# Chrissie-Law/Causal-Domain-Clustering-for-Multi-Domain-Recommendation

Hardware: AMD Instinct MI355X
Metric: train samples/sec + AUC parity, PLE 3-domain batch 4096 at 1/2/4/8 MI355X (higher is better)
Workload: dtype bf16; 1 GPU; PLE 3-domain full training step (fwd + BCE + whole-table L2 + bwd + Adam), 26 fields x vocab 1000000, emb_dim=16, batch 4096/GPU; global_batch=4096, table_mode=lazy, hip_graph=True, row_sort_one_batch_ahead=True, id_dist=uniform, parallelism=dp1, attention_branch=False, full=False, steady_state=True, preroll_steps=1785, flush_every=64

## Files before the change

causal-domain-clustering-for-multi-domain-recommendation_amd/_lib.py:

```python
import ctypes as C
import os

from . import build as _build

MAX_GROUPS = 32
MAX_TENSORS = 48
MAX_GATES = 16
MAX_SEL = 16
MAX_BN_SEGS = 24
SORT_MAX_B = 16384
SORT_MAX_ROWS = 32768
BN_ROWS_PER_BLOCK = 64
ROWDOT_PARTS = 256
PREC_BF16 = 0
PREC_F32 = 1

c_f = C.c_float
c_d = C.c_double
c_i32 = C.c_int32
c_i64 = C.c_int64
c_p = C.c_void_p


class AdamHP(C.Structure):
# ... 176 lines not shown

class MidBExpert2(C.Structure):
    _fields_ = [("wt", c_p), ("ldwt", c_i64), ("src", c_i32), ("pad_", c_i32)]


class MidBGate2(C.Structure):
    _fields_ = [("d_out", c_p), ("ld_dout", c_i64), ("probs", c_p), ("d_logits", c_p), ("ld_dlogits", c_i64),
                ("d_logits_h", c_p), ("ld_dlogits_h", c_i64), ("wt", c_p), ("ldwt", c_i64), ("src", c_i32), ("n_sel", c_i32),
                ("sel", c_i32 * MAX_SEL)]


class CgcMidBwdArgs(C.Structure):
    _fields_ = [("B", c_i64), ("H1", c_i32), ("H2", c_i32), ("n_exp1", c_i32), ("n_gate1", c_i32), ("n_exp2", c_i32), ("n_gate2", c_i32),
                ("ex1", c_p), ("ld_ex1", c_i64), ("ex2", c_p), ("ld_ex2", c_i64), ("dz1_h", c_p), ("ld_dz1_h", c_i64),
                ("dz2_h", c_p), ("ld_dz2_h", c_i64), ("mask1", c_i32), ("mask2", c_i32), ("scale1", c_f), ("scale2", c_f),
                ("g1", MidBGate1 * MID_MAX_GATE), ("e2", MidBExpert2 * MID_MAX_EXPERT), ("g2", MidBGate2 * MID_MAX_GATE)]


BN_X_BF16, BN_Y_BF16, BN_DY_BF16 = 1, 2, 4


class BnSeg(C.Structure):
    _fields_ = [("x", c_p), ("ldx", c_i64), ("y", c_p), ("ldy", c_i64), ("gamma", c_p), ("beta", c_p),
                ("running_mean", c_p), ("running_var", c_p), ("save_mean", c_p), ("save_invstd", c_p),
                ("num_batches_tracked", c_p), ("yh", c_p), ("ldyh", c_i64), ("C", c_i32), ("row_group", c_i32),
                ("half", c_i32), ("pad_", c_i32)]


class BnFwdArgs(C.Structure):
    _fields_ = [("n_seg", c_i32), ("training", c_i32), ("relu", c_i32), ("skip_le1", c_i32), ("eps", c_f), ("momentum", c_f),
                ("drop_p", c_f), ("seed", C.c_uint64), ("seed_offset_dev", c_p), ("M", c_i64),
                ("row_offsets", c_p), ("workspace", c_p), ("phase", c_i32), ("stats_ready", c_i32), ("exchange", c_p),
                ("s", BnSeg * MAX_BN_SEGS)]


class BnBSeg(C.Structure):
    _fields_ = [("dy", c_p), ("lddy", c_i64), ("y", c_p), ("ldy", c_i64), ("x", c_p), ("ldx", c_i64),
                ("dx", c_p), ("lddx", c_i64), ("gamma", c_p), ("save_mean", c_p), ("save_invstd", c_p),
                ("dgamma", c_p), ("dbeta", c_p), ("dxh", c_p), ("lddxh", c_i64), ("C", c_i32), ("row_group", c_i32), ("accumulate_dx", c_i32),
                ("half", c_i32)]


class BnBwdArgs(C.Structure):
    _fields_ = [("n_seg", c_i32), ("training", c_i32), ("relu", c_i32), ("eps", c_f), ("mask_scale", c_f),
                ("M", c_i64), ("row_offsets", c_p), ("workspace", c_p), ("phase", c_i32), ("pad_", c_i32), ("exchange", c_p),
                ("s", BnBSeg * MAX_BN_SEGS)]


class RowdotGroup(C.Structure):
    _fields_ = [("x", c_p), ("ldx", c_i64), ("w", c_p), ("bias", c_p), ("out", c_p), ("ld_out", c_i64),
                ("logit", c_p), ("ld_logit", c_i64), ("K", c_i32)]


class RowdotFwdArgs(C.Structure):
    _fields_ = [("n_groups", c_i32), ("sigmoid", c_i32), ("n_addend", c_i32), ("addend", c_p * 4),
                ("ld_addend", c_i64 * 4), ("M", c_i64), ("row_offsets", c_p), ("g", RowdotGroup * MAX_GROUPS)]


class RowdotBGroup(C.Structure):
    _fields_ = [("dout", c_p), ("ld_dout", c_i64), ("out", c_p), ("ld_out", c_i64), ("x", c_p), ("ldx", c_i64),
                ("w", c_p), ("dx", c_p), ("lddx", c_i64), ("dw", c_p), ("dbias", c_p), ("dlogit", c_p),
                ("ld_dlogit", c_i64), ("K", c_i32), ("accumulate_dx", c_i32)]


class RowdotBwdArgs(C.Structure):
    _fields_ = [("n_groups", c_i32), ("sigmoid", c_i32), ("M", c_i64), ("row_offsets", c_p), ("workspace", c_p),
                ("bce_group", c_p), ("bce_y_i16", c_p), ("bce_y_f32", c_p), ("bce_loss", c_p), ("bce_partial", c_p),
                ("bce_inv_count", c_f), ("pad_", c_i32), ("g", RowdotBGroup * MAX_GROUPS)]


HEAD_MAX_TOWERS = 8


class HeadTower(C.Structure):
    _fields_ = [("x", c_p), ("ldx", c_i64), ("w", c_p), ("bias", c_p), ("dx", c_p), ("lddx", c_i64), ("dw", c_p), ("dbias", c_p),
                ("K", c_i32), ("accumulate_dx", c_i32)]


class HeadArgs(C.Structure):
    _fields_ = [("n_tower", c_i32), ("sigmoid", c_i32), ("n_addend", c_i32), ("pad_", c_i32), ("M", c_i64),
                ("out", c_p), ("ld_out", c_i64), ("d_out", c_p), ("ld_dout", c_i64),
                ("wide_x", c_p), ("ld_wide", c_i64), ("wide_w", c_p), ("wide_bias", c_p), ("wide_out", c_p), ("ld_wide_out", c_i64),
                ("wide_dx", c_p), ("ld_wide_dx", c_i64), ("wide_dw", c_p), ("wide_dbias", c_p), ("wide_K", c_i32), ("accumulate_wide_dx", c_i32),
                ("addend", c_p * 2), ("ld_addend", c_i64 * 2), ("d_addend", c_p * 2), ("ld_d_addend", c_i64 * 2),
                ("accumulate_d_addend", c_i32 * 2), ("workspace", c_p),
                ("bce_group", c_p), ("bce_y_i16", c_p), ("bce_y_f32", c_p), ("bce_loss", c_p), ("bce_partial", c_p),
                ("bce_inv_count", c_f), ("pad2_", c_i32), ("t", HeadTower * HEAD_MAX_TOWERS)]


TOWER_MAX = 4
TOWER_ROWS = 128
TOWER_ERR_TIMEOUT = 0x40000000


class TowerLayer(C.Structure):
    _fields_ = [("wh", c_p), ("ldwh", c_i64), ("wt", c_p), ("ldwt", c_i64), ("bias", c_p), ("z", c_p), ("ldz", c_i64),
                ("dzh", c_p), ("lddzh", c_i64), ("gamma", c_p), ("beta", c_p), ("running_mean", c_p), ("running_var", c_p),
                ("num_batches_tracked", c_p), ("save_mean", c_p), ("save_invstd", c_p), ("dgamma", c_p), ("dbeta", c_p)]


class TowerDesc(C.Structure):
    _fields_ = [("xh", c_p), ("ldxh", c_i64), ("dx", c_p), ("lddx", c_i64), ("accumulate_dx", c_i32), ("pad_", c_i32),
                ("l1", TowerLayer), ("l2", TowerLayer), ("a1h", c_p), ("lda1h", c_i64), ("a2", c_p), ("lda2", c_i64),
                ("wo", c_p), ("bo", c_p), ("dwo", c_p), ("dbo", c_p), ("dy2", c_p), ("lddy2", c_i64), ("dy1", c_p), ("lddy1", c_i64)]


class TowerArgs(C.Structure):
    _fields_ = [("n_tower", c_i32), ("H0", c_i32), ("H1", c_i32), ("H2", c_i32), ("M", c_i64), ("relu", c_i32), ("sigmoid", c_i32),
                ("drop_p", c_f), ("eps", c_f), ("momentum", c_f), ("pad_", c_i32), ("seed1", C.c_uint64), ("seed2", C.c_uint64),
                ("seed_offset_dev", c_p), ("out", c_p), ("ld_out", c_i64), ("d_out", c_p), ("ld_dout", c_i64),
                ("wide_x", c_p), ("ld_wide", c_i64), ("wide_w", c_p), ("wide_bias", c_p), ("wide_dx", c_p), ("ld_wide_dx", c_i64),
                ("wide_dw", c_p), ("wide_dbias", c_p), ("wide_K", c_i32), ("accumulate_wide_dx", c_i32),
                ("bce_group", c_p), ("bce_y_i16", c_p), ("bce_y_f32", c_p), ("bce_loss", c_p), ("bce_inv_count", c_f), ("pad2_", c_i32),
                ("workspace", c_p), ("err", c_p), ("exchange", c_p * 4), ("t", TowerDesc * TOWER_MAX)]


class StarFuseArgs(C.Structure):
    _fields_ = [("n", c_i32), ("op", c_i32), ("size", c_i64), ("s", c_p), ("ds", c_p), ("accumulate_ds", c_i32), ("pad_", c_i32),
                ("a", c_p * MAX_GROUPS), ("out", c_p * MAX_GROUPS), ("da", c_p * MAX_GROUPS)]


class AdamTensor(C.Structure):
    _fields_ = [("w", c_p), ("g", c_p), ("m", c_p), ("v", c_p), ("n", c_i64), ("l2", c_f), ("n_slabs", c_i32), ("slabs", c_p),
                ("slab_stride", c_i64)]


class AddNArgs(C.Structure):
    _fields_ = [("dst", c_p), ("ld_dst", c_i64), ("rows", c_i64), ("cols", c_i32), ("n", c_i32), ("accumulate", c_i32),
                ("src", c_p * MAX_GROUPS), ("ld_src", c_i64 * MAX_GROUPS)]


class AdamArgs(C.Structure):
    _fields_ = [("n_tensors", c_i32), ("lerp_w", c_f), ("beta2", c_f), ("one_minus_beta2", c_f), ("eps", c_f),
                ("weight_decay", c_f), ("step_scalars", c_p), ("n_scalars", c_i32), ("grad_scale", c_f),
                ("step_dev", c_p), ("reg_sum", c_p), ("reg_seed", c_p), ("t", AdamTensor * MAX_TENSORS)]


_SIGNATURES = {
    "cdc_abi_version": (c_i32, []),
    "cdc_last_error": (C.c_char_p, []),
    "cdc_embed_gather_fwd": (c_i32, [c_p, c_p, c_p, c_p, c_p, c_p, c_i64, c_i32, c_i32, c_i64, c_p]),
    "cdc_embed_gather_fwd_h": (c_i32, [c_p, c_p, c_p, c_p, c_p, c_i64, c_p, c_p, c_i64, c_i32, c_i32, c_i64, c_p]),
    "cdc_embed_index": (c_i32, [c_p, c_p, c_p, c_p, c_i64, c_i32, c_i64, c_p]),
    "cdc_embed_sort_dedupe": (c_i32, [c_p, c_p, c_p, c_p, c_p, c_p, c_i64, c_i32, c_p]),
    "cdc_embed_sort_dedupe_ids": (c_i32, [c_p, c_p, c_i64, c_p, c_p, c_i32, c_p, c_p, c_p, c_p, c_p, c_p, c_i64, c_i32, c_p]),
    "cdc_embed_segment_sum": (c_i32, [c_p, c_p, c_p, c_p, c_p, c_p, c_i64, c_i32, c_i32, c_p]),
    "cdc_embed_segment_sum_direct": (c_i32, [c_p, c_p, c_p, c_p, c_p, c_p, c_i64, c_i32, c_i32, c_p]),
    "cdc_embed_segsum_lazy_update": (c_i32, [c_p, c_p, c_p, c_p, c_p, c_p, c_p, c_p, c_p, AdamHP, c_p, c_i64, c_i32, c_i32, c_i32, c_p]),
    "cdc_embed_grad_dense": (c_i32, [c_p, c_p, c_p, c_p, c_i64, c_i32, c_i32, c_i64, c_p]),
    "cdc_embed_adam_touched": (c_i32, [c_p, c_p, c_p, c_p, c_p, c_p, c_p, AdamHP, c_p, c_i64, c_i32, c_i32, c_p]),
    "cdc_embed_adam_dense_pass": (c_i32, [c_p, c_p, c_p, c_i64, AdamHP, c_p, c_p, c_p]),
    "cdc_embed_adam_patch": (c_i32, [c_p, c_p, c_p, c_p, c_p, c_p, c_i64, c_i32, c_i32, c_p]),
    "cdc_embed_lazy_catchup": (c_i32, [c_p, c_p, c_p, c_p, c_p, c_p, AdamHP, c_p, c_p, c_i32, c_i64, c_i32, c_i32, c_p]),
    "cdc_embed_lazy_catchup_gather": (c_i32, [c_p, c_p, c_p, c_p, c_p, c_p, c_p, c_p, AdamHP, c_p, c_p, c_p, c_i64, c_i64, c_i32, c_i32, c_p]),
    "cdc_embed_lazy_update": (c_i32, [c_p, c_p, c_p, c_p, c_p, c_p, c_p, AdamHP, c_p, c_p, c_i32, c_i64, c_i32, c_i32, c_p]),
    "cdc_embed_lazy_flush": (c_i32, [c_p, c_p, c_p, c_p, c_i64, c_i32, AdamHP, c_p, c_i32, c_i32, c_i32, c_i32, c_p]),
    "cdc_embed_lazy_flush_bg": (c_i32, [c_p, c_p, c_p, c_p, c_i64, c_i32, AdamHP, c_p, c_i32, c_i32, c_i32, c_i32, c_i32, c_p]),
    "cdc_embed_merge_dedupe": (c_i32, [c_p, c_p, c_p, c_p, c_p, c_p, c_i64, c_i32, c_i32, c_p]),
    "cdc_eval_workspace_bytes": (c_i64, [c_i64, c_i32]),
    "cdc_eval_metrics": (c_i32, [c_p, c_p, c_p, c_i64, c_i64, c_i32, c_p, c_p, c_p, c_p, c_i64, c_p]),
    "cdc_eval_gauc_workspace_bytes": (c_i64, [c_i64, c_i32, c_i64]),
    "cdc_eval_gauc": (c_i32, [c_p, c_p, c_p, c_i64, c_i64, c_p, c_i64, c_i32, c_p, c_i64, c_p, c_p, c_p, c_p, c_i64, c_p]),
    "cdc_eval_auc_delong_workspace_bytes": (c_i64, [c_i64, c_i32, c_i32]),
    "cdc_eval_auc_delong": (c_i32, [c_p, c_p, c_p, c_p, c_i64, c_i64, c_i32, c_p, c_p, c_p, c_p, c_i64, c_p]),
    "cdc_eval_loss_ci_workspace_bytes": (c_i64, [c_i64, c_i32, c_i32]),
    "cdc_eval_loss_ci": (c_i32, [c_p, c_p, c_p, c_p, c_i64, c_i64, c_i32, c_p, c_p, c_p, c_p, c_i64, c_p]),
    "cdc_eval_gauc_ci_workspace_bytes": (c_i64, [c_i64, c_i32, c_i64, c_i32]),
    "cdc_eval_gauc_ci": (c_i32, [c_p, c_p, c_p, c_p, c_i64, c_i64, c_p, c_i64, c_i32, c_p, c_i64, c_p, c_p, c_p, c_p, c_i64, c_p]),
    "cdc_eval_bootstrap_workspace_bytes": (c_i64, [c_i64, c_i32, c_i64, c_i32, c_i32]),
    "cdc_eval_bootstrap": (c_i32, [c_p, c_p, c_p, c_p, c_i64, c_i64, c_p, c_i64, c_i32, c_p, c_i64, c_i32, C.c_uint64, c_i32, c_p, c_p, c_p,
                                   c_p, c_i64, c_p]),
    "cdc_eval_calibration_bootstrap_workspace_bytes": (c_i64, [c_i64, c_i32, c_i32, c_i32, c_i32]),
    "cdc_eval_calibration_bootstrap": (c_i32, [c_p, c_p, c_p, c_p, c_i64, c_i64, c_p, c_i64, c_i32, c_i32, c_i64, c_i32, C.c_uint64, c_p,
                                               c_p, c_p, c_p, c_i64, c_p]),
    "cdc_eval_calibration_workspace_bytes": (c_i64, [c_i64, c_i32, c_i32]),
    "cdc_eval_calibration": (c_i32, [c_p, c_p, c_p, c_i64, c_i64, c_i32, c_i32, c_p, c_p, c_p, c_p, c_p, c_p, c_p, c_i64, c_p]),
    "cdc_eval_isotonic_max_blocks": (c_i64, [c_i64, c_i32]),
    "cdc_eval_isotonic_fit_workspace_bytes": (c_i64, [c_i64, c_i32]),
    "cdc_eval_isotonic_fit": (c_i32, [c_p, c_p, c_p, c_i64, c_i64, c_i32, c_p, c_p, c_p, c_p, c_p, c_p, c_i64, c_p, c_p, c_p, c_p, c_i64, c_p]),
    "cdc_eval_isotonic_apply": (c_i32, [c_p, c_p, c_i64, c_i64, c_i32, c_p, c_p, c_p, c_p, c_p, c_f, c_p, c_p, c_p]),
    "cdc_eval_platt_fit_workspace_bytes": (c_i64, [c_i64, c_i32]),
    "cdc_eval_platt_fit": (c_i32, [c_p, c_p, c_p, c_i64, c_i64, c_i32, c_i32, c_i32, c_d, c_d, c_i32, c_p, c_p, c_p, c_p, c_p, c_p, c_p, c_p, c_p, c_p,
                                   c_p, c_i64, c_p]),
    "cdc_eval_platt_apply": (c_i32, [c_p, c_p, c_i64, c_i64, c_i32, c_p, c_p, c_p, c_i32, c_d, c_f, c_p, c_p, c_p]),
    "cdc_eval_segments": (c_i32, [c_p, c_i64, c_p, c_p, c_i32, c_p, c_p, c_p, c_p, c_p, c_i64, c_i32, c_p]),
    "cdc_shard_bucket": (c_i32, [c_p, c_p, c_p, c_p, c_p, c_i64, c_i32, c_i32, c_i32, c_p]),
    "cdc_shard_expand": (c_i32, [c_p, c_p, c_p, c_p, c_p, c_p, c_p, c_i64, c_i32, c_i32, c_i32, c_i32, c_p]),
    "cdc_shard_pack": (c_i32, [c_p, c_p, c_p, c_p, c_p, c_i64, c_i32, c_i32, c_i32, c_i32, c_p]),
    "cdc_glinear_fwd": (c_i32, [C.POINTER(LinFwdArgs), c_i32, c_p]),
    "cdc_glinear_bwd_x": (c_i32, [C.POINTER(LinBwdxArgs), c_i32, c_p]),
    "cdc_transpose_multi": (c_i32, [C.POINTER(TransposeArgs), c_p]),
    "cdc_gemm_bf16_nt": (c_i32, [C.POINTER(G2Args), c_p]),
    "cdc_weight_shadows": (c_i32, [C.POINTER(WShadowArgs), c_p]),
    "cdc_shadow_bf16": (c_i32, [C.POINTER(ShadowArgs), c_p]),
    "cdc_glinear_bwd_w": (c_i32, [C.POINTER(LinBwdwArgs), c_i32, c_p]),
    "cdc_glinear_bwd_w_pair": (c_i32, [C.POINTER(LinBwdwArgs), C.POINTER(LinBwdwArgs), c_p, c_p]),
    "cdc_glinear_bwd_w_pair_reduce": (c_i32, [C.POINTER(LinBwdwArgs), C.POINTER(LinBwdwArgs), c_p, c_p]),
    "cdc_gate_pool_fwd": (c_i32, [C.POINTER(PoolFwdArgs), c_p]),
    "cdc_cgc_mid_fwd": (c_i32, [C.POINTER(CgcMidFwdArgs), c_p]),
    "cdc_cgc_mid_bwd": (c_i32, [C.POINTER(CgcMidBwdArgs), c_p]),
    "cdc_cgc_mid_fits": (c_i32, [c_i32, c_i32, c_i32, c_i32]),
    "cdc_expert_pair_fwd": (c_i32, [C.POINTER(ExpertPairArgs), c_p]),
    "cdc_gate_pool_bwd": (c_i32, [C.POINTER(PoolBwdArgs), c_p]),
    "cdc_gate_pool_wide_table": (c_i32, [c_i32, c_i32, c_p, c_p, c_p, c_i64]),
    "cdc_gate_pool_wide_fwd": (c_i32, [C.POINTER(PoolWideFwdArgs), c_p]),
    "cdc_gate_pool_wide_bwd": (c_i32, [C.POINTER(PoolWideBwdArgs), c_p]),
    "cdc_bn_fwd": (c_i32, [C.POINTER(BnFwdArgs), c_p]),
    "cdc_bn_bwd": (c_i32, [C.POINTER(BnBwdArgs), c_p]),
    "cdc_rowdot_fwd": (c_i32, [C.POINTER(RowdotFwdArgs), c_p]),
    "cdc_rowdot_bwd": (c_i32, [C.POINTER(RowdotBwdArgs), c_p]),
    "cdc_head_fwd": (c_i32, [C.POINTER(HeadArgs), c_p]),
    "cdc_head_bwd": (c_i32, [C.POINTER(HeadArgs), c_p]),
    "cdc_head_workspace_floats": (c_i64, [C.POINTER(HeadArgs)]),
    "cdc_tower_fwd": (c_i32, [C.POINTER(TowerArgs), c_p]),
    "cdc_tower_bwd": (c_i32, [C.POINTER(TowerArgs), c_p]),
    "cdc_tower_step": (c_i32, [C.POINTER(TowerArgs), c_p]),
    "cdc_tower_workspace_bytes": (c_i64, [C.POINTER(TowerArgs)]),
    "cdc_tower_dp": (c_i32, [C.POINTER(TowerArgs), c_i32, c_p]),
    "cdc_bce_fwd_bwd": (c_i32, [c_p, c_i64, c_p, c_p, c_p, c_p, c_p, c_i64, c_i64, c_i32, c_f, c_p]),
    "cdc_attn_fwd": (c_i32, [c_p, c_i64, c_p, c_i64, c_p, c_i64, c_i32, c_i32, c_i32, c_f, C.c_uint64, c_p, c_p]),
    "cdc_attn_bwd": (c_i32, [c_p, c_i64, c_p, c_p, c_i64, c_p, c_i64, c_i64, c_i32, c_i32, c_i32, c_f, C.c_uint64, c_p, c_p]),
    "cdc_add_relu_fwd": (c_i32, [c_p, c_i64, c_p, c_i64, c_p, c_i64, c_i64, c_i32, c_p]),
    "cdc_add_relu_bwd": (c_i32, [c_p, c_i64, c_p, c_i64, c_p, c_i64, c_i32, c_p, c_i64, c_i32, c_i64, c_i32, c_p]),
    "cdc_sigmoid_gate_fwd": (c_i32, [c_p, c_i64, c_p, c_i64, c_p, c_i64, c_i64, c_i32, c_f, c_f, c_f, c_p]),
    "cdc_sigmoid_gate_bwd": (c_i32, [c_p, c_i64, c_p, c_i64, c_p, c_i64, c_p, c_i64, c_i32, c_p, c_i64, c_i32, c_i64, c_i32, c_f, c_f, c_f, c_p]),
    "cdc_group_select_fwd": (c_i32, [c_p, c_i64, c_p, c_p, c_i64, c_i64, c_i32, c_i32, c_p]),
    "cdc_group_select_bwd": (c_i32, [c_p, c_i64, c_p, c_p, c_i64, c_i64, c_i32, c_i32, c_i32, c_p]),
    "cdc_stage_batch": (c_i32, [c_p, c_p, c_p, c_p, c_p, c_p, c_i64, c_i32, c_p, c_p, c_p]),
    "cdc_stage_batch_next": (c_i32, [c_p, c_p, c_p, c_p, c_p, c_p, c_i64, c_i32, c_p, c_p, c_p, c_p, c_i32, c_p, c_p, c_p]),
    "cdc_fm_fwd": (c_i32, [c_p, c_i64, c_p, c_i64, c_i64, c_i32, c_i32, c_p]),
    "cdc_fm_bwd": (c_i32, [c_p, c_i64, c_p, c_i64, c_p, c_i64, c_i64, c_i32, c_i32, c_i32, c_p]),
    "cdc_bce_mean_fwd_bwd": (c_i32, [c_p, c_i64, c_p, c_p, c_p, c_p, c_i64, c_i64, c_i32, c_f, c_p]),
    "cdc_cross_fwd": (c_i32, [c_p, c_i64, c_p, c_i64, c_p, c_p, c_p, c_i64, c_p, c_i64, c_i32, c_p]),
    "cdc_cross_bwd": (c_i32, [c_p, c_i64, c_p, c_i64, c_p, c_i64, c_p, c_p, c_p, c_i64, c_p, c_i64, c_p, c_p, c_p, c_i64, c_i32, c_p]),
    "cdc_tanh_fwd": (c_i32, [c_p, c_i64, c_p, c_i64, c_i64, c_i32, c_p]),
    "cdc_tanh_bwd": (c_i32, [c_p, c_i64, c_p, c_i64, c_p, c_i64, c_i64, c_i32, c_i32, c_p]),
    "cdc_cross_combine_fwd": (c_i32, [c_p, c_i64, c_p, c_i64, c_p, c_p, c_p, c_i64, c_p, c_i64, c_i64, c_i32, c_i32, c_p]),
    "cdc_cross_combine_bwd": (c_i32, [c_p, c_i64, c_p, c_i64, c_p, c_i64, c_p, c_p, c_i64, c_p, c_i64, c_p, c_i64, c_i32,
                                      c_p, c_i32, c_p, c_i32, c_p, c_i64, c_i32, c_i32, c_p]),
    "cdc_add_out": (c_i32, [c_p, c_i64, c_p, c_i64, c_p, c_i64, c_i64, c_i32, c_p]),
    "cdc_copy_or_add": (c_i32, [c_p, c_i64, c_p, c_i64, c_i64, c_i32, c_i32, c_p]),
    "cdc_star_fuse_fwd": (c_i32, [C.POINTER(StarFuseArgs), c_p]),
    "cdc_star_fuse_bwd": (c_i32, [C.POINTER(StarFuseArgs), c_p]),
    "cdc_sum_slices": (c_i32, [c_p, c_i64, c_p, c_i64, c_i64, c_i32, c_i32, c_i32, c_p]),
    "cdc_adam_multi": (c_i32, [C.POINTER(AdamArgs), c_p]),
    "cdc_adam_multi_table": (c_i32, [C.POINTER(AdamArgs), c_p, c_p, c_p, c_i32, c_p]),
    "cdc_embed_segsum_lazy_update_dense": (c_i32, [c_p, c_p, c_p, c_p, c_p, c_p, c_p, c_p, c_p, AdamHP, c_p, c_i64, c_i32, c_i32, c_i32,
                                                   C.POINTER(AdamArgs), c_p, c_p, c_p, c_i32, c_p]),
    "cdc_step_increment": (c_i32, [c_p, c_p]),
    "cdc_begin_step": (c_i32, [c_p, c_p, c_i32, c_p]),
    "cdc_fill_f32": (c_i32, [c_p, c_f, c_i64, c_p]),
    "cdc_fill_f64": (c_i32, [c_p, C.c_double, c_i64, c_p]),
    "cdc_add_inplace": (c_i32, [c_p, c_i64, c_p, c_i64, c_i64, c_i32, c_p]),
    "cdc_add_n": (c_i32, [c_p, c_p]),
    "cdc_mul_bcast": (c_i32, [c_p, c_p, c_p, c_i64, c_i64, c_p]),
    "cdc_mul_bcast_bwd": (c_i32, [c_p, c_p, c_p, c_p, c_p, c_i64, c_i64, c_p]),
    "cdc_group_partition": (c_i32, [c_p, c_p, c_p, c_i64, c_i32, c_p]),
    "cdc_rows_permute": (c_i32, [c_p, c_i64, c_p, c_p, c_i64, c_i64, c_i32, c_i32, c_p]),
}

_lib = None


class HipExtensionError(RuntimeError):
    pass


def lib_path():
    return _build.LIB_PATH


def load():
    global _lib
    if _lib is not None:
        return _lib
    path = _build.LIB_PATH
    if not _build.is_fresh():
        try:
            _build.build(verbose=False)
        except Exception as e:
            if not os.path.exists(path):
                raise HipExtensionError(
                    f"libcdcmdr.so is missing at {path} and could not be built ({e}); "
                    "run `python __graft_entry__.py build` — there is no CPU fallback") from e
            import warnings
            warnings.warn(f"libcdcmdr.so is older than its sources and the rebuild failed: {str(e)[:400]}")
    try:
        lib = C.CDLL(path)
    except OSError as e:
        raise HipExtensionError(f"cannot load {path}: {e}; there is no CPU fallback") from e
    for name, (res, args) in _SIGNATURES.items():
        try:
            fn = getattr(lib, name)
        except AttributeError as e:
            raise HipExtensionError(f"{path} does not export {name}") from e
        fn.restype = res
        fn.argtypes = args
    if lib.cdc_abi_version() != 1:
        raise HipExtensionError(f"ABI version mismatch: library {lib.cdc_abi_version()} != binding 1")
    _lib = lib
    return lib


def exported_symbols():
    return sorted(_SIGNATURES)


def check(rc, what):
    if rc != 0:
        msg = load().cdc_last_error()
        raise RuntimeError(f"{what} failed (rc={rc}): {msg.decode() if msg else ''}")


PROFILE = None
TRACE = os.environ.get("CDC_TRACE_LAUNCH") == "1"


def launch(name, fn, args, stream, flops=0.0, nbytes=0.0):
    if TRACE:
        import sys
        sys.stderr.write(f"[cdc launch] {name}\n")
        sys.stderr.flush()
    if PROFILE is None:
        rc = fn(*args, stream)
    else:
        import torch
        e0, e1 = torch.cuda.Event(enable_timing=True), torch.cuda.Event(enable_timing=True)
        e0.record()
        rc = fn(*args, stream)
        e1.record()
        PROFILE.append((name, e0, e1, flops, nbytes))
    if rc != 0:
        check(rc, name)
```

causal-domain-clustering-for-multi-domain-recommendation_amd/csrc/embedding.hip:

```cpp
#include "common.h"
#include "adam_dense.h"

template <int VEC>
__global__ void __launch_bounds__(256) k_gather_fwd(const int32_t* __restrict__ ids, const int32_t* __restrict__ offsets,
                                                    const float* __restrict__ table, float* __restrict__ out,
                                                    __bf16* __restrict__ out_h, int64_t ld_out_h,
                                                    int32_t* __restrict__ idx_out, int32_t* __restrict__ err_flag,
                                                    int64_t n_pos, int32_t F, int32_t D, int64_t R) {
    CDC_PRIO_MAIN();
    const int chunks = D / VEC;
    const int64_t total = n_pos * chunks;
    for (int64_t i = (int64_t)blockIdx.x * blockDim.x + threadIdx.x; i < total; i += (int64_t)gridDim.x * blockDim.x) {
        const int64_t pos = i / chunks;
        const int c = (int)(i - pos * chunks);
        const int f = (int)(pos % F);
        const int32_t row = (int32_t)((uint32_t)ids[pos] + (uint32_t)offsets[f]);
        const bool ok = row >= 0 && (int64_t)row < R;
        if (c == 0 && idx_out) idx_out[pos] = ok ? row : -1;
        if (!ok && c == 0 && err_flag) atomicMax(err_flag, (int32_t)(pos < 0x7ffffffe ? pos + 1 : 0x7fffffff));
        if (VEC == 4) {
            float4 val = make_float4(0.f, 0.f, 0.f, 0.f);
            if (ok) val = *reinterpret_cast<const float4*>(table + (int64_t)row * D + c * 4);
            *reinterpret_cast<float4*>(out + pos * D + c * 4) = val;
            if (out_h) {
// ... 406 lines not shown
static int sort_raise_lds_limit(const char* who) {
    static bool attr_set = false;
    if (attr_set) return 0;
    const void* const kernels[] = {(const void*)k_sort_dedupe, (const void*)k_sort_chunk, (const void*)k_merge_lds<uint64_t, false>,
                                   (const void*)k_merge_lds<uint32_t, true>};
    for (const void* k : kernels) {
        const hipError_t e = hipFuncSetAttribute(k, hipFuncAttributeMaxDynamicSharedMemorySize, 160 * 1024);
        if (e != hipSuccess) { cdc_set_error("%s: cannot raise LDS limit: %s", who, hipGetErrorString(e)); return (int)e; }
    }
    attr_set = true;
    return 0;
}
static int merge_lanes(const char* who, int n_runs, int& P) {
    P = 1;
    while (P < n_runs) P <<= 1;
    CDC_CHECK_ARG(P <= 64, CDC_E_TOOBIG, "%s: %d runs", who, n_runs);
    return 0;
}
static int dedupe_merged_launch(const uint64_t* merged, int32_t* uniq_row, int32_t* seg_start, int32_t* perm, int32_t* uniq_cnt, int64_t B,
                                int32_t F, hipStream_t st) {
    hipLaunchKernelGGL(k_dedupe_merged, dim3(F), dim3(SORT_THREADS), 0, st, merged, uniq_row, seg_start, perm, uniq_cnt, (int32_t)B, F);
    CDC_LAUNCH_CHECK("embed_dedupe_merged");
    return 0;
}

static int sort_dedupe_launch(const SortSrc& src, int32_t* uniq_row, int32_t* seg_start, int32_t* perm, int32_t* uniq_cnt,
                              uint64_t* scratch, int64_t B, int32_t F, void* stream) {
    const int32_t* idx = src.idx;
    CDC_CHECK_ARG(idx && uniq_row && seg_start && perm && uniq_cnt, CDC_E_BADARG, "embed_sort_dedupe: null pointer");
    CDC_CHECK_ARG(B > 0 && F > 0, CDC_E_BADARG, "embed_sort_dedupe: bad sizes");
    CDC_CHECK_ARG(B <= CDC_SORT_MAX_ROWS, CDC_E_TOOBIG, "embed_sort_dedupe: B=%ld exceeds %d", (long)B, CDC_SORT_MAX_ROWS);
    CDC_CHECK_ARG(scratch || B <= SORT_CHUNK, CDC_E_BADARG, "embed_sort_dedupe: B > %d needs a scratch buffer of 2*F*B uint64", SORT_CHUNK);
    if (const int rc = sort_raise_lds_limit("embed_sort_dedupe")) return rc;
    hipStream_t st = (hipStream_t)stream;
    if (B > 1024 && B <= SORT_RADIX_MAX) {
        hipLaunchKernelGGL(k_sort_dedupe_radix, dim3(F), dim3(SORT_THREADS), 0, st, src, uniq_row, seg_start, perm, uniq_cnt, (int32_t)B, F);
        CDC_LAUNCH_CHECK("embed_sort_dedupe_radix");
        return 0;
    }
    if (B <= 1024 || (!scratch && B <= SORT_CHUNK)) {
        int n_pad = SORT_THREADS;
        while (n_pad < B) n_pad <<= 1;
        const size_t lds = (size_t)n_pad * 8 + SORT_THREADS * 4;
        hipLaunchKernelGGL(k_sort_dedupe, dim3(F), dim3(SORT_THREADS), lds, st, src, uniq_row, seg_start, perm, uniq_cnt, (int32_t)B, F, n_pad);
        CDC_LAUNCH_CHECK("embed_sort_dedupe");
        return 0;
    }
    int chunk = 512;
    while (chunk < SORT_CHUNK && (int64_t)chunk * 8 < B) chunk <<= 1;
    const int n_runs = (int)cdc_ceil_div(B, chunk);
    uint64_t* runs = scratch;
    uint64_t* merged = scratch + (int64_t)F * B;
    hipLaunchKernelGGL(k_sort_chunk, dim3(F, n_runs), dim3(SORT_THREADS), (size_t)chunk * 8, st, src, runs, (int32_t)B, F, chunk);
    CDC_LAUNCH_CHECK("embed_sort_chunk");
    int P;
    if (const int rc = merge_lanes("embed_sort_dedupe", n_runs, P)) return rc;
    if ((size_t)B * 8 <= MERGE_LDS_MAX) {
        hipLaunchKernelGGL((k_merge_lds<uint64_t, false>), dim3(F, n_runs), dim3(SORT_THREADS), (size_t)B * 8, st, runs, merged, (int32_t)B, F,
                           n_runs, chunk, P);
    } else {
        const int64_t blocks = cdc_ceil_div((int64_t)F * B * P, 256);
        hipLaunchKernelGGL(k_merge_runs, dim3((unsigned)blocks), dim3(256), 0, st, runs, merged, (int32_t)B, F, chunk, n_runs, P);
    }
    CDC_LAUNCH_CHECK("embed_merge_runs");
    return dedupe_merged_launch(merged, uniq_row, seg_start, perm, uniq_cnt, B, F, st);
}

extern "C" int cdc_embed_sort_dedupe(const int32_t* idx, int32_t* uniq_row, int32_t* seg_start, int32_t* perm,
                                     int32_t* uniq_cnt, uint64_t* scratch, int64_t B, int32_t F, void* stream) {
    const SortSrc src = {idx, nullptr, 0, nullptr, nullptr, 0, nullptr};
    return sort_dedupe_launch(src, uniq_row, seg_start, perm, uniq_cnt, scratch, B, F, stream);
}
extern "C" int cdc_embed_sort_dedupe_ids(const int32_t* ids, const int32_t* offsets, int64_t R, int32_t* step_dev, double* accumulators,
                                         int32_t n_acc, int32_t* err_flag, int32_t* uniq_row, int32_t* seg_start, int32_t* perm,
                                         int32_t* uniq_cnt, uint64_t* scratch, int64_t B, int32_t F, void* stream) {
    CDC_CHECK_ARG(offsets && R > 0 && n_acc >= 0 && n_acc <= 64 && (n_acc == 0 || accumulators) && (step_dev || n_acc == 0), CDC_E_BADARG,
                  "embed_sort_dedupe_ids: bad argument");
    const SortSrc src = {ids, offsets, R, step_dev, accumulators, n_acc, err_flag};
    return sort_dedupe_launch(src, uniq_row, seg_start, perm, uniq_cnt, scratch, B, F, stream);
}

extern "C" int cdc_embed_merge_dedupe(const int32_t* idx, int32_t* uniq_row, int32_t* seg_start, int32_t* perm, int32_t* uniq_cnt,
                                      uint64_t* scratch, int64_t B, int32_t F, int32_t n_runs, void* stream) {
    CDC_CHECK_ARG(idx && uniq_row && seg_start && perm && uniq_cnt && scratch, CDC_E_BADARG, "embed_merge_dedupe: null pointer");
    CDC_CHECK_ARG(B > 0 && F > 0 && n_runs > 0 && B % n_runs == 0, CDC_E_BADARG, "embed_merge_dedupe: bad sizes");
    CDC_CHECK_ARG(B <= CDC_SORT_MAX_ROWS, CDC_E_TOOBIG, "embed_merge_dedupe: B=%ld exceeds %d", (long)B, CDC_SORT_MAX_ROWS);
    hipStream_t st = (hipStream_t)stream;
    int P;
    if (const int rc = merge_lanes("embed_merge_dedupe", n_runs, P)) return rc;
    if (const int rc = sort_raise_lds_limit("embed_merge_dedupe")) return rc;
    static_assert((size_t)CDC_SORT_MAX_ROWS * 4 <= MERGE_LDS_MAX, "cdc_embed_merge_dedupe stages a whole field in LDS");
    hipLaunchKernelGGL((k_merge_lds<uint32_t, true>), dim3(F, n_runs), dim3(SORT_THREADS), (size_t)B * 4, st, idx, scratch, (int32_t)B, F,
                       n_runs, (int32_t)(B / n_runs), P);
    CDC_LAUNCH_CHECK("embed_merge_n");
    return dedupe_merged_launch(scratch, uniq_row, seg_start, perm, uniq_cnt, B, F, st);
}

struct RowItem {
    int64_t slot, row;
    int f, j, d;
    bool live;
};
template <int VEC, bool ROW = true>
__device__ __forceinline__ RowItem row_item(int64_t i, int chunks, int B, const int32_t* __restrict__ uniq_cnt,
                                            const int32_t* __restrict__ uniq_row) {
    RowItem it;
    it.d = (int)(i % chunks) * VEC;
    it.slot = i / chunks;
    it.f = (int)(it.slot / B);
    it.j = (int)(it.slot - (int64_t)it.f * B);
    it.row = -1;
    it.live = it.j < uniq_cnt[it.f];
    if (ROW && it.live) {
        it.row = uniq_row[it.slot];
        it.live = it.row >= 0;
    }
    return it;
}
template <int VEC>
__device__ __forceinline__ void load_wmv(const float* w, const float* m, const float* v, int64_t e0, float (&wv)[VEC], float (&mv)[VEC],
                                         float (&vv)[VEC]) {
    if (VEC == 4) {
        const float4 a4 = *reinterpret_cast<const float4*>(w + e0), b4 = *reinterpret_cast<const float4*>(m + e0),
                     c4 = *reinterpret_cast<const float4*>(v + e0);
        wv[0] = a4.x; wv[1 % VEC] = a4.y; wv[2 % VEC] = a4.z; wv[3 % VEC] = a4.w;
        mv[0] = b4.x; mv[1 % VEC] = b4.y; mv[2 % VEC] = b4.z; mv[3 % VEC] = b4.w;
        vv[0] = c4.x; vv[1 % VEC] = c4.y; vv[2 % VEC] = c4.z; vv[3 % VEC] = c4.w;
    } else {
        wv[0] = w[e0]; mv[0] = m[e0]; vv[0] = v[e0];
    }
}
template <int VEC>
__device__ __forceinline__ void store_wmv(float* w, float* m, float* v, int64_t e0, const float (&wv)[VEC], const float (&mv)[VEC],
                                          const float (&vv)[VEC]) {
    if (VEC == 4) {
        *reinterpret_cast<float4*>(w + e0) = make_float4(wv[0], wv[1 % VEC], wv[2 % VEC], wv[3 % VEC]);
        *reinterpret_cast<float4*>(m + e0) = make_float4(mv[0], mv[1 % VEC], mv[2 % VEC], mv[3 % VEC]);
        *reinterpret_cast<float4*>(v + e0) = make_float4(vv[0], vv[1 % VEC], vv[2 % VEC], vv[3 % VEC]);
    } else {
        w[e0] = wv[0]; m[e0] = mv[0]; v[e0] = vv[0];
    }
}
template <int VEC>
__device__ __forceinline__ void row_adam_step(float* w, float* m, float* v, int32_t* last, int64_t row, int D, int d0, const float (&g)[VEC],
                                              const AdamConsts& c, float step_size, float bc2s, int32_t t) {
    const int64_t e0 = row * D + d0;
    float wv[VEC], mv[VEC], vv[VEC];
    load_wmv<VEC>(w, m, v, e0, wv, mv, vv);
#pragma unroll
    for (int q = 0; q < VEC; ++q) adam_elem(wv[q], mv[q], vv[q], g[q], c, step_size, bc2s);
    store_wmv<VEC>(w, m, v, e0, wv, mv, vv);
    if (d0 == 0) last[row] = t;
}

#define SEG_SPLIT 64
#define SEG_DIRECT 8
#define SEG_BLOCK 512
#define SEG_LONG_BLOCKS 64
#define SEG_LIST_CAP (CDC_SORT_MAX_ROWS / SEG_LONG_BLOCKS)

struct SegSink {
    float* rowgrad;
    float* w; float* m; float* v;
    int32_t* last;
    const int32_t* uniq_row;
    AdamConsts c;
    float step_size, bc2s;
    int32_t t;
};
template <int VEC>
__device__ __forceinline__ void seg_finish(const SegSink& k, int64_t slot, int D, int d0, const float (&acc)[VEC]) {
    if (!k.w) {
        float* dst = k.rowgrad + slot * D + d0;
        if (VEC == 4) *reinterpret_cast<float4*>(dst) = make_float4(acc[0], acc[1 % VEC], acc[2 % VEC], acc[3 % VEC]);
        else dst[0] = acc[0];
        return;
    }
    const int64_t row = k.uniq_row[slot];
    if (row < 0) return;
    row_adam_step<VEC>(k.w, k.m, k.v, k.last, row, D, d0, acc, k.c, k.step_size, k.bc2s, k.t);
}
__device__ __forceinline__ SegSink seg_sink_store(float* rowgrad) {
    SegSink k = {};
    k.rowgrad = rowgrad;
    return k;
}

template <int VEC>
__device__ __forceinline__ void seg_direct_body(int bid, int nblocks, const float* __restrict__ d_out, const int32_t* __restrict__ seg_start,
                                                const int32_t* __restrict__ perm, const int32_t* __restrict__ uniq_cnt,
                                                const int32_t* __restrict__ uniq_row, const SegSink& sink,
                                                int32_t B, int32_t F, int32_t D, int32_t max_len) {
    const int chunks = D / VEC;
    const int64_t total = (int64_t)F * B * chunks;
    for (int64_t i = (int64_t)bid * blockDim.x + threadIdx.x; i < total; i += (int64_t)nblocks * blockDim.x) {
        const RowItem it = row_item<VEC, false>(i, chunks, B, uniq_cnt, nullptr);
        if (!it.live) continue;
        if (uniq_row && uniq_row[it.slot] < 0) continue;
        const int f = it.f, j = it.j;
        const int32_t* sst = seg_start + (int64_t)f * (B + 1);
        const int32_t* prm = perm + (int64_t)f * B;
        const int k0 = sst[j], k1 = sst[j + 1];
        if (max_len > 0 && k1 - k0 >= max_len) continue;
        float acc[VEC];
#pragma unroll
        for (int q = 0; q < VEC; ++q) acc[q] = 0.f;
        for (int k = k0; k < k1; k += 8) {
            int p[8];
            float v[8][VEC];
#pragma unroll
            for (int q = 0; q < 8; ++q) p[q] = (k + q < k1) ? prm[k + q] : -1;
#pragma unroll
            for (int q = 0; q < 8; ++q) {
                const float* src = d_out + ((int64_t)(p[q] >= 0 ? p[q] : 0) * F + f) * D + it.d;
                if (p[q] >= 0) {
                    if (VEC == 4) {
                        const float4 t = *reinterpret_cast<const float4*>(src);
                        v[q][0] = t.x; v[q][1] = t.y; v[q][2] = t.z; v[q][3] = t.w;
                    } else {
                        v[q][0] = src[0];
                    }
                }
            }
#pragma unroll
            for (int q = 0; q < 8; ++q)
                if (p[q] >= 0) {
#pragma unroll
                    for (int e = 0; e < VEC; ++e) acc[e] = __fadd_rn(acc[e], v[q][e]);
                }
        }
        seg_finish<VEC>(sink, it.slot, D, it.d, acc);
    }
}
template <int VEC>
__global__ void __launch_bounds__(256) k_segment_sum_direct(const float* __restrict__ d_out, const int32_t* __restrict__ seg_start,
                                                            const int32_t* __restrict__ perm, const int32_t* __restrict__ uniq_cnt,
                                                            const int32_t* __restrict__ uniq_row, float* __restrict__ rowgrad,
                                                            int32_t B, int32_t F, int32_t D, int32_t max_len) {
    seg_direct_body<VEC>(blockIdx.x, gridDim.x, d_out, seg_start, perm, uniq_cnt, uniq_row, seg_sink_store(rowgrad), B, F, D, max_len);
}
extern "C" int cdc_embed_segment_sum_direct(const float* d_out, const int32_t* seg_start, const int32_t* perm,
                                            const int32_t* uniq_cnt, const int32_t* uniq_row, float* rowgrad, int64_t B, int32_t F,
                                            int32_t D, void* stream) {
    CDC_CHECK_ARG(d_out && seg_start && perm && uniq_cnt && rowgrad, CDC_E_BADARG, "embed_segment_sum_direct: null pointer");
    CDC_CHECK_ARG(B > 0 && F > 0 && D > 0 && B <= CDC_SORT_MAX_ROWS, CDC_E_BADARG, "embed_segment_sum_direct: bad sizes");
    const bool vec = (D % 4 == 0) && (((uintptr_t)d_out | (uintptr_t)rowgrad) % 16 == 0);
    int blocks = (int)std::min<int64_t>(cdc_ceil_div((int64_t)F * B * (vec ? D / 4 : D), 256), 8192);
    if (vec)
        hipLaunchKernelGGL(k_segment_sum_direct<4>, dim3(blocks), dim3(256), 0, (hipStream_t)stream, d_out, seg_start, perm, uniq_cnt, uniq_row,
                           rowgrad, (int32_t)B, F, D, 0);
    else
        hipLaunchKernelGGL(k_segment_sum_direct<1>, dim3(blocks), dim3(256), 0, (hipStream_t)stream, d_out, seg_start, perm, uniq_cnt, uniq_row,
                           rowgrad, (int32_t)B, F, D, 0);
    CDC_LAUNCH_CHECK("embed_segment_sum_direct");
    return 0;
}

template <int BATCH = 16>
__device__ __forceinline__ float seg_serial_sum(const float* __restrict__ d_out, const int32_t* __restrict__ prm, int begin, int end,
                                                int F, int D, int f, int d) {
    float acc = 0.f;
    for (int k = begin; k < end; k += BATCH) {
        int p[BATCH];
        float x[BATCH];
#pragma unroll
        for (int q = 0; q < BATCH; ++q) p[q] = (k + q < end) ? prm[k + q] : -1;
#pragma unroll
        for (int q = 0; q < BATCH; ++q) x[q] = p[q] >= 0 ? d_out[((int64_t)p[q] * F + f) * D + d] : 0.f;
#pragma unroll
        for (int q = 0; q < BATCH; ++q)
            if (p[q] >= 0) acc = __fadd_rn(acc, x[q]);
    }
    return acc;
}
template <int VEC>
__device__ __forceinline__ void seg_long_body(int f, int by, const float* __restrict__ d_out, const int32_t* __restrict__ seg_start,
                                              const int32_t* __restrict__ perm, const int32_t* __restrict__ uniq_cnt,
                                              const SegSink& sink, int32_t B, int32_t F, int32_t D, int32_t subs,
                                              int32_t min_len) {
    __shared__ int32_t list[SEG_LIST_CAP];
    __shared__ int32_t n_list;
    __shared__ __attribute__((aligned(16))) float parts[256 * VEC];
    const int tid = threadIdx.x, lane = tid & 63, wave = tid >> 6;
    const int n = uniq_cnt[f];
    const int32_t* sst = seg_start + (int64_t)f * (B + 1);
    const int32_t* prm = perm + (int64_t)f * B;
    if (tid == 0) n_list = 0;
    __syncthreads();
    for (int j = by + SEG_LONG_BLOCKS * tid; j < n; j += SEG_LONG_BLOCKS * 256)
        if (sst[j + 1] - sst[j] >= min_len) list[atomicAdd(&n_list, 1)] = j;
    __syncthreads();
    const int count = n_list;
    if (count == 0) return;
    const bool block_rows = subs > 1;
    for (int i = wave; i < count; i += 4) {
        const int j = list[i];
        const int k0 = sst[j], len = sst[j + 1] - k0;
        if (block_rows && len >= SEG_BLOCK) continue;
        const int64_t slot = (int64_t)f * B + j;
        if (subs <= 1) {
            for (int d = lane; d < D; d += 64) {
                const float one[1] = {seg_serial_sum(d_out, prm + k0, 0, len, F, D, f, d)};
                seg_finish<1>(sink, slot, D, d, one);
            }
            continue;
        }
        const int sub = lane / D, d = lane - sub * D;
        const bool split = len >= SEG_SPLIT;
        int begin = 0, end = (sub == 0) ? len : 0;
        if (split) {
            const int q = (len + subs - 1) / subs;
            begin = min(sub * q, len);
            end = min(begin + q, len);
        }
        float acc = seg_serial_sum(d_out, prm + k0, begin, end, F, D, f, d);
        if (split) {
            float total = __shfl(acc, d, 64);
            for (int s2 = 1; s2 < subs; ++s2) total = __fadd_rn(total, __shfl(acc, s2 * D + d, 64));
            acc = total;
        }
        if (sub == 0) {
            const float one[1] = {acc};
            seg_finish<1>(sink, slot, D, d, one);
        }
    }
    if (!block_rows) return;
    const int chunks = D / VEC;
    const int P = 256 / chunks;
    const int part = tid / chunks, d = (tid - part * chunks) * VEC;
    for (int i = 0; i < count; ++i) {
        const int j = list[i];
        const int k0 = sst[j], len = sst[j + 1] - k0;
        if (len < SEG_BLOCK) continue;
        const int q = (len + P - 1) / P;
        const int begin = min(part * q, len), end = min(begin + q, len);
        float acc[VEC];
#pragma unroll
        for (int e = 0; e < VEC; ++e) acc[e] = 0.f;
        if (part < P) {
            constexpr int NB = VEC == 4 ? 16 : 32;
            for (int k = begin; k < end; k += NB) {
                int pr[NB];
#pragma unroll
                for (int u = 0; u < NB; ++u) pr[u] = (k + u < end) ? prm[k0 + k + u] : -1;
                float x[NB][VEC];
#pragma unroll
                for (int u = 0; u < NB; ++u) {
                    if (pr[u] >= 0) {
                        const float* src = d_out + ((int64_t)pr[u] * F + f) * D + d;
                        if (VEC == 4) {
                            const float4 t4 = *reinterpret_cast<const float4*>(src);
                            x[u][0] = t4.x; x[u][1 % VEC] = t4.y; x[u][2 % VEC] = t4.z; x[u][3 % VEC] = t4.w;
                        } else {
                            x[u][0] = src[0];
                        }
                    }
                }
#pragma unroll
                for (int u = 0; u < NB; ++u)
                    if (pr[u] >= 0) {
#pragma unroll
                        for (int e = 0; e < VEC; ++e) acc[e] = __fadd_rn(acc[e], x[u][e]);
                    }
            }
        }
#pragma unroll
        for (int e = 0; e < VEC; ++e) parts[tid * VEC + e] = acc[e];
        __syncthreads();
        if (tid < chunks) {
            float total[VEC];
#pragma unroll
            for (int e = 0; e < VEC; ++e) total[e] = parts[tid * VEC + e];
            for (int p2 = 1; p2 < P; ++p2)
#pragma unroll
                for (int e = 0; e < VEC; ++e) total[e] = __fadd_rn(total[e], parts[(p2 * chunks + tid) * VEC + e]);
            seg_finish<VEC>(sink, (int64_t)f * B + j, D, tid * VEC, total);
        }
        __syncthreads();
    }
}

template <int VEC>
__global__ void __launch_bounds__(256) k_segment_sum(const float* __restrict__ d_out, const int32_t* __restrict__ seg_start,
                                                     const int32_t* __restrict__ perm, const int32_t* __restrict__ uniq_cnt,
                                                     SegSink sink, cdc_adam_hp hp, const int32_t* __restrict__ step_dev, int32_t B,
                                                     int32_t F, int32_t D, int32_t subs) {
    if (sink.w) {
        sink.c = make_consts(hp);
        sink.t = *step_dev;
        step_scalars_at(hp.step_scalars, hp.n_scalars, sink.t, sink.step_size, sink.bc2s);
    }
    const int n_long = F * SEG_LONG_BLOCKS;
    if ((int)blockIdx.x < n_long)
        seg_long_body<VEC>(blockIdx.x / SEG_LONG_BLOCKS, blockIdx.x % SEG_LONG_BLOCKS, d_out, seg_start, perm, uniq_cnt, sink, B, F, D,
                           subs, SEG_DIRECT);
    else
        seg_direct_body<VEC>(blockIdx.x - n_long, gridDim.x - n_long, d_out, seg_start, perm, uniq_cnt, nullptr, sink, B, F, D, SEG_DIRECT);
}
template <int VEC>
__global__ void __launch_bounds__(256, 4) k_segment_sum_dense(const float* __restrict__ d_out, const int32_t* __restrict__ seg_start,
                                                           const int32_t* __restrict__ perm, const int32_t* __restrict__ uniq_cnt,
                                                           SegSink sink, cdc_adam_hp hp, const int32_t* __restrict__ step_dev, int32_t B,
                                                           int32_t F, int32_t D, int32_t subs, const AdamHdr h,
                                                           const cdc_adam_tensor* __restrict__ tab, const int32_t* __restrict__ wg_tensor,
                                                           const int32_t* __restrict__ wg_chunk, int32_t n_dense, int32_t short_only) {
    const int n_long = short_only ? 0 : F * SEG_LONG_BLOCKS;
    const int b = (int)blockIdx.x;
    if (b >= n_long && b < n_long + n_dense) {
        const int ti = __builtin_amdgcn_readfirstlane(wg_tensor[b - n_long]);
        const int chunk = __builtin_amdgcn_readfirstlane(wg_chunk[b - n_long]);
        const cdc_adam_tensor T = tab[ti];
        adam_chunk<ADAM_CHUNK / 2>(h, T, chunk, b == n_long);
        return;
    }
    sink.c = make_consts(hp);
    sink.t = *step_dev;
    step_scalars_at(hp.step_scalars, hp.n_scalars, sink.t, sink.step_size, sink.bc2s);
    if (b < n_long)
        seg_long_body<VEC>(b / SEG_LONG_BLOCKS, b % SEG_LONG_BLOCKS, d_out, seg_start, perm, uniq_cnt, sink, B, F, D, subs, SEG_DIRECT);
    else
        seg_direct_body<VEC>(b - n_long - n_dense, (int)gridDim.x - n_long - n_dense, d_out, seg_start, perm, uniq_cnt,
                             short_only ? sink.uniq_row : nullptr, sink, B, F, D, short_only ? 0 : SEG_DIRECT);
}
template <int VEC>
__global__ void __launch_bounds__(256) k_segment_sum_short_sink(const float* __restrict__ d_out, const int32_t* __restrict__ seg_start,
                                                                const int32_t* __restrict__ perm, const int32_t* __restrict__ uniq_cnt,
                                                                SegSink sink, cdc_adam_hp hp, const int32_t* __restrict__ step_dev,
                                                                int32_t B, int32_t F, int32_t D) {
    sink.c = make_consts(hp);
    sink.t = *step_dev;
    step_scalars_at(hp.step_scalars, hp.n_scalars, sink.t, sink.step_size, sink.bc2s);
    seg_direct_body<VEC>(blockIdx.x, gridDim.x, d_out, seg_start, perm, uniq_cnt, sink.uniq_row, sink, B, F, D, 0);
}

struct SegGeom {
    bool vec;
    int direct_blocks, subs;
    SegSink sink;
};
static SegGeom seg_geometry(const float* d_out, float* rowgrad, float* w, float* m, float* v, int32_t* last, const int32_t* uniq_row,
                            int64_t B, int32_t F, int32_t D) {
    SegGeom g = {};
    g.vec = (D % 4 == 0) && (((uintptr_t)d_out | (uintptr_t)rowgrad | (uintptr_t)w | (uintptr_t)m | (uintptr_t)v) % 16 == 0);
    g.direct_blocks = (int)std::min<int64_t>(cdc_ceil_div((int64_t)F * B * (g.vec ? D / 4 : D), 256), 8192);
    g.subs = (D <= 64 && 64 % D == 0) ? 64 / D : 1;
    g.sink.rowgrad = rowgrad;
    g.sink.w = w; g.sink.m = m; g.sink.v = v; g.sink.last = last; g.sink.uniq_row = uniq_row;
    return g;
}

extern "C" int cdc_embed_segment_sum(const float* d_out, const int32_t* seg_start, const int32_t* perm,
                                     const int32_t* uniq_cnt, float* sorted_scratch, float* rowgrad, int64_t B, int32_t F,
                                     int32_t D, void* stream) {
    (void)sorted_scratch;
    CDC_CHECK_ARG(d_out && seg_start && perm && uniq_cnt && rowgrad, CDC_E_BADARG, "embed_segment_sum: null pointer");
    CDC_CHECK_ARG(B > 0 && F > 0 && D > 0 && B <= CDC_SORT_MAX_ROWS, CDC_E_BADARG, "embed_segment_sum: bad sizes");
    hipStream_t st = (hipStream_t)stream;
    const SegGeom g = seg_geometry(d_out, rowgrad, nullptr, nullptr, nullptr, nullptr, nullptr, B, F, D);
    const int blocks = g.direct_blocks + F * SEG_LONG_BLOCKS;
    const cdc_adam_hp no_hp = {};
    if (g.vec) hipLaunchKernelGGL(k_segment_sum<4>, dim3(blocks), dim3(256), 0, st, d_out, seg_start, perm, uniq_cnt, g.sink, no_hp, nullptr, (int32_t)B, F, D, g.subs);
    else       hipLaunchKernelGGL(k_segment_sum<1>, dim3(blocks), dim3(256), 0, st, d_out, seg_start, perm, uniq_cnt, g.sink, no_hp, nullptr, (int32_t)B, F, D, g.subs);
    CDC_LAUNCH_CHECK("embed_segment_sum");
    return 0;
}

extern "C" int cdc_embed_segsum_lazy_update(const float* d_out, const int32_t* seg_start, const int32_t* perm, const int32_t* uniq_cnt,
                                            const int32_t* uniq_row, float* w, float* m, float* v, int32_t* last, cdc_adam_hp hp,
                                            const int32_t* step_dev, int64_t B, int32_t F, int32_t D, int32_t short_only, void* stream) {
    CDC_CHECK_ARG(d_out && seg_start && perm && uniq_cnt && uniq_row && w && m && v && last && step_dev && hp.step_scalars &&
                      hp.n_scalars > 0, CDC_E_BADARG, "embed_segsum_lazy_update: null pointer");
    CDC_CHECK_ARG(B > 0 && F > 0 && D > 0 && B <= CDC_SORT_MAX_ROWS, CDC_E_BADARG, "embed_segsum_lazy_update: bad sizes");
    hipStream_t st = (hipStream_t)stream;
    const SegGeom g = seg_geometry(d_out, nullptr, w, m, v, last, uniq_row, B, F, D);
    if (short_only) {
        if (g.vec) hipLaunchKernelGGL(k_segment_sum_short_sink<4>, dim3(g.direct_blocks), dim3(256), 0, st, d_out, seg_start, perm, uniq_cnt, g.sink, hp, step_dev, (int32_t)B, F, D);
        else       hipLaunchKernelGGL(k_segment_sum_short_sink<1>, dim3(g.direct_blocks), dim3(256), 0, st, d_out, seg_start, perm, uniq_cnt, g.sink, hp, step_dev, (int32_t)B, F, D);
    } else {
        const int blocks = g.direct_blocks + F * SEG_LONG_BLOCKS;
        if (g.vec) hipLaunchKernelGGL(k_segment_sum<4>, dim3(blocks), dim3(256), 0, st, d_out, seg_start, perm, uniq_cnt, g.sink, hp, step_dev, (int32_t)B, F, D, g.subs);
        else       hipLaunchKernelGGL(k_segment_sum<1>, dim3(blocks), dim3(256), 0, st, d_out, seg_start, perm, uniq_cnt, g.sink, hp, step_dev, (int32_t)B, F, D, g.subs);
    }
    CDC_LAUNCH_CHECK("embed_segsum_lazy_update");
    return 0;
}

extern "C" int cdc_embed_segsum_lazy_update_dense(const float* d_out, const int32_t* seg_start, const int32_t* perm, const int32_t* uniq_cnt,
                                                  const int32_t* uniq_row, float* w, float* m, float* v, int32_t* last, cdc_adam_hp hp,
                                                  const int32_t* step_dev, int64_t B, int32_t F, int32_t D, int32_t short_only,
                                                  const cdc_adam_args* dense, const cdc_adam_tensor* tensors_dev, const int32_t* wg_tensor_dev,
                                                  const int32_t* wg_chunk_dev, int32_t n_dense_workgroups, void* stream) {
    CDC_CHECK_ARG(d_out && seg_start && perm && uniq_cnt && uniq_row && w && m && v && last && step_dev && hp.step_scalars &&
                      hp.n_scalars > 0, CDC_E_BADARG, "embed_segsum_lazy_update_dense: null pointer");
    CDC_CHECK_ARG(B > 0 && F > 0 && D > 0 && B <= CDC_SORT_MAX_ROWS, CDC_E_BADARG, "embed_segsum_lazy_update_dense: bad sizes");
    CDC_CHECK_ARG(dense && tensors_dev && wg_tensor_dev && wg_chunk_dev && n_dense_workgroups > 0 && n_dense_workgroups < (1 << 24) &&
                      dense->step_dev && dense->step_scalars && dense->n_scalars > 0, CDC_E_BADARG,
                  "embed_segsum_lazy_update_dense: the dense parameters' descriptor table (as for cdc_adam_multi_table) is missing");
    hipStream_t st = (hipStream_t)stream;
    const SegGeom g = seg_geometry(d_out, nullptr, w, m, v, last, uniq_row, B, F, D);
    const int blocks = g.direct_blocks + (short_only ? 0 : F * SEG_LONG_BLOCKS) + n_dense_workgroups;
    const AdamHdr h = {dense->lerp_w, dense->beta2, dense->one_minus_beta2, dense->eps, dense->weight_decay, dense->grad_scale,
                       dense->step_scalars, dense->n_scalars, dense->step_dev, dense->reg_sum, dense->reg_seed};
    if (g.vec) hipLaunchKernelGGL(k_segment_sum_dense<4>, dim3(blocks), dim3(256), 0, st, d_out, seg_start, perm, uniq_cnt, g.sink, hp, step_dev, (int32_t)B, F, D, g.subs,
                                  h, tensors_dev, wg_tensor_dev, wg_chunk_dev, n_dense_workgroups, short_only);
    else       hipLaunchKernelGGL(k_segment_sum_dense<1>, dim3(blocks), dim3(256), 0, st, d_out, seg_start, perm, uniq_cnt, g.sink, hp, step_dev, (int32_t)B, F, D, g.subs,
                                  h, tensors_dev, wg_tensor_dev, wg_chunk_dev, n_dense_workgroups, short_only);
    CDC_LAUNCH_CHECK("embed_segsum_lazy_update_dense");
    return 0;
}

__global__ void __launch_bounds__(256) k_grad_dense(const float* __restrict__ rowgrad, const int32_t* __restrict__ uniq_row,
                                                    const int32_t* __restrict__ uniq_cnt, float* __restrict__ grad,
                                                    int32_t B, int32_t F, int32_t D, int64_t R) {
    const int64_t total = (int64_t)F * B * D;
    for (int64_t i = (int64_t)blockIdx.x * blockDim.x + threadIdx.x; i < total; i += (int64_t)gridDim.x * blockDim.x) {
        const RowItem it = row_item<1>(i, D, B, uniq_cnt, uniq_row);
        if (!it.live || it.row >= R) continue;
        grad[it.row * D + it.d] += rowgrad[i];
    }
}

extern "C" int cdc_embed_grad_dense(const float* rowgrad, const int32_t* uniq_row, const int32_t* uniq_cnt, float* grad,
                                    int64_t B, int32_t F, int32_t D, int64_t R, void* stream) {
    CDC_CHECK_ARG(rowgrad && uniq_row && uniq_cnt && grad, CDC_E_BADARG, "embed_grad_dense: null pointer");
    CDC_CHECK_ARG(B > 0 && F > 0 && D > 0 && B <= CDC_SORT_MAX_ROWS, CDC_E_BADARG, "embed_grad_dense: bad sizes");
    const int64_t total = (int64_t)F * B * D;
    int blocks = (int)std::min<int64_t>(cdc_ceil_div(total, 256), 256 * 16);
    hipLaunchKernelGGL(k_grad_dense, dim3(blocks), dim3(256), 0, (hipStream_t)stream, rowgrad, uniq_row, uniq_cnt, grad,
                       (int32_t)B, F, D, R);
    CDC_LAUNCH_CHECK("embed_grad_dense");
    return 0;
}

__global__ void __launch_bounds__(256) k_adam_touched(const float* __restrict__ rowgrad, const int32_t* __restrict__ uniq_row,
                                                      const int32_t* __restrict__ uniq_cnt, const float* __restrict__ w,
                                                      const float* __restrict__ m, const float* __restrict__ v,
                                                      float* __restrict__ side, cdc_adam_hp hp,
                                                      const int32_t* __restrict__ step_dev, int32_t B, int32_t F, int32_t D) {
    const AdamConsts c = make_consts(hp);
    float step_size, bc2s;
    step_scalars_at(hp.step_scalars, hp.n_scalars, *step_dev, step_size, bc2s);
    const int64_t total = (int64_t)F * B * D;
    for (int64_t i = (int64_t)blockIdx.x * blockDim.x + threadIdx.x; i < total; i += (int64_t)gridDim.x * blockDim.x) {
        const RowItem it = row_item<1>(i, D, B, uniq_cnt, uniq_row);
        if (!it.live) continue;
        const int d = it.d;
        float wv = w[it.row * D + d], mv = m[it.row * D + d], vv = v[it.row * D + d];
        adam_elem(wv, mv, vv, rowgrad[i], c, step_size, bc2s);
        float* s = side + it.slot * 3 * D;
        s[d] = wv; s[D + d] = mv; s[2 * D + d] = vv;
    }
}

extern "C" int cdc_embed_adam_touched(const float* rowgrad, const int32_t* uniq_row, const int32_t* uniq_cnt, const float* w,
                                      const float* m, const float* v, float* side, cdc_adam_hp hp, const int32_t* step_dev,
                                      int64_t B, int32_t F, int32_t D, void* stream) {
    CDC_CHECK_ARG(rowgrad && uniq_row && uniq_cnt && w && m && v && side && step_dev && hp.step_scalars, CDC_E_BADARG,
                  "embed_adam_touched: null pointer");
    CDC_CHECK_ARG(B > 0 && F > 0 && D > 0 && B <= CDC_SORT_MAX_ROWS && hp.n_scalars > 0, CDC_E_BADARG, "embed_adam_touched: bad sizes");
    const int64_t total = (int64_t)F * B * D;
    int blocks = (int)std::min<int64_t>(cdc_ceil_div(total, 256), 256 * 16);
    hipLaunchKernelGGL(k_adam_touched, dim3(blocks), dim3(256), 0, (hipStream_t)stream, rowgrad, uniq_row, uniq_cnt, w, m, v, side,
                       hp, step_dev, (int32_t)B, F, D);
    CDC_LAUNCH_CHECK("embed_adam_touched");
    return 0;
}

__global__ void __launch_bounds__(256) k_adam_dense_pass(float* __restrict__ w, float* __restrict__ m, float* __restrict__ v,
                                                         int64_t n_vec4, int64_t n_elems, cdc_adam_hp hp,
                                                         const int32_t* __restrict__ step_dev, double* __restrict__ reg_sum) {
    const AdamConsts c = make_consts(hp);
    float step_size, bc2s;
    step_scalars_at(hp.step_scalars, hp.n_scalars, *step_dev, step_size, bc2s);
    double sq = 0.0;
    const int64_t stride = (int64_t)gridDim.x * blockDim.x;
    for (int64_t i = (int64_t)blockIdx.x * blockDim.x + threadIdx.x; i < n_vec4; i += stride) {
        float4 wv = reinterpret_cast<float4*>(w)[i];
        float4 mv = reinterpret_cast<float4*>(m)[i];
        float4 vv = reinterpret_cast<float4*>(v)[i];
        sq += (double)(wv.x * wv.x + wv.y * wv.y) + (double)(wv.z * wv.z + wv.w * wv.w);
        adam_elem(wv.x, mv.x, vv.x, 0.f, c, step_size, bc2s);
        adam_elem(wv.y, mv.y, vv.y, 0.f, c, step_size, bc2s);
        adam_elem(wv.z, mv.z, vv.z, 0.f, c, step_size, bc2s);
        adam_elem(wv.w, mv.w, vv.w, 0.f, c, step_size, bc2s);
        reinterpret_cast<float4*>(w)[i] = wv;
        reinterpret_cast<float4*>(m)[i] = mv;
        reinterpret_cast<float4*>(v)[i] = vv;
    }
    for (int64_t i = n_vec4 * 4 + (int64_t)blockIdx.x * blockDim.x + threadIdx.x; i < n_elems; i += stride) {
        float wv = w[i], mv = m[i], vv = v[i];
        sq += (double)(wv * wv);
        adam_elem(wv, mv, vv, 0.f, c, step_size, bc2s);
        w[i] = wv; m[i] = mv; v[i] = vv;
    }
    if (reg_sum) {
        __shared__ double part[4];
        sq = wave_sum_d(sq);
        if ((threadIdx.x & 63) == 0) part[threadIdx.x >> 6] = sq;
        __syncthreads();
        if (threadIdx.x == 0) atomicAdd(reg_sum, part[0] + part[1] + part[2] + part[3]);
    }
}

extern "C" int cdc_embed_adam_dense_pass(float* w, float* m, float* v, int64_t n_elems, cdc_adam_hp hp,
                                         const int32_t* step_dev, double* reg_sum, void* stream) {
    CDC_CHECK_ARG(w && m && v && step_dev && hp.step_scalars && hp.n_scalars > 0, CDC_E_BADARG, "embed_adam_dense_pass: null pointer");
    CDC_CHECK_ARG(n_elems > 0, CDC_E_BADARG, "embed_adam_dense_pass: bad size");
    CDC_CHECK_ARG((((uintptr_t)w | (uintptr_t)m | (uintptr_t)v) % 16) == 0, CDC_E_ALIGN, "embed_adam_dense_pass: buffers must be 16-byte aligned");
    const int64_t n_vec4 = n_elems / 4;
    int blocks = (int)std::min<int64_t>(std::max<int64_t>(cdc_ceil_div(n_vec4, 256), 1), 256 * 8);
    hipLaunchKernelGGL(k_adam_dense_pass, dim3(blocks), dim3(256), 0, (hipStream_t)stream, w, m, v, n_vec4, n_elems, hp,
                       step_dev, reg_sum);
    CDC_LAUNCH_CHECK("embed_adam_dense_pass");
    return 0;
}

__global__ void __launch_bounds__(256) k_adam_patch(const float* __restrict__ side, const int32_t* __restrict__ uniq_row,
                                                    const int32_t* __restrict__ uniq_cnt, float* __restrict__ w,
                                                    float* __restrict__ m, float* __restrict__ v, int32_t B, int32_t F,
                                                    int32_t D) {
    const int64_t total = (int64_t)F * B * D;
    for (int64_t i = (int64_t)blockIdx.x * blockDim.x + threadIdx.x; i < total; i += (int64_t)gridDim.x * blockDim.x) {
        const RowItem it = row_item<1>(i, D, B, uniq_cnt, uniq_row);
        if (!it.live) continue;
        const int d = it.d;
        const float* s = side + it.slot * 3 * D;
        w[it.row * D + d] = s[d];
        m[it.row * D + d] = s[D + d];
        v[it.row * D + d] = s[2 * D + d];
    }
}

extern "C" int cdc_embed_adam_patch(const float* side, const int32_t* uniq_row, const int32_t* uniq_cnt, float* w,
                                    float* m, float* v, int64_t B, int32_t F, int32_t D, void* stream) {
    CDC_CHECK_ARG(side && uniq_row && uniq_cnt && w && m && v, CDC_E_BADARG, "embed_adam_patch: null pointer");
    CDC_CHECK_ARG(B > 0 && F > 0 && D > 0, CDC_E_BADARG, "embed_adam_patch: bad sizes");
    const int64_t total = (int64_t)F * B * D;
    int blocks = (int)std::min<int64_t>(cdc_ceil_div(total, 256), 256 * 16);
    hipLaunchKernelGGL(k_adam_patch, dim3(blocks), dim3(256), 0, (hipStream_t)stream, side, uniq_row, uniq_cnt, w, m, v,
                       (int32_t)B, F, D);
    CDC_LAUNCH_CHECK("embed_adam_patch");
    return 0;
}

template <bool FAST, int VEC>
__global__ void __launch_bounds__(256) k_lazy_catchup(const int32_t* __restrict__ uniq_row, const int32_t* __restrict__ uniq_cnt,
                                                      float* __restrict__ w, float* __restrict__ m, float* __restrict__ v,
                                                      int32_t* __restrict__ last, cdc_adam_hp hp,
                                                      const int32_t* __restrict__ step_dev, int32_t B, int32_t F, int32_t D,
                                                      int32_t mark) {
    const AdamConsts c = make_consts(hp);
    const int target = *step_dev - 1;
    const int chunks = D / VEC;
    const int64_t total = (int64_t)F * B * chunks;
    for (int64_t base = (int64_t)blockIdx.x * blockDim.x; base < total; base += (int64_t)gridDim.x * blockDim.x) {
        const int64_t i = base + threadIdx.x;
        bool act = i < total;
        int d = 0, from = target;
        int64_t row = -1;
        if (act) {
            const RowItem it = row_item<VEC>(i, chunks, B, uniq_cnt, uniq_row);
            d = it.d;
            row = it.row;
            act = it.live;
        }
        if (act) from = last[row];
        act = act && from < target;
        if (!act) from = target;
        if (!__any(act)) continue;
        const int64_t e0 = act ? row * D + d : 0;
        float wv[VEC], mv[VEC], vv[VEC];
#pragma unroll
        for (int k = 0; k < VEC; ++k) { wv[k] = 0.f; mv[k] = 0.f; vv[k] = 1.f; }
        if (act) load_wmv<VEC>(w, m, v, e0, wv, mv, vv);
        adam_replay_wave<FAST, VEC>(wv, mv, vv, from, target, c, hp);
        if (!act) continue;
        store_wmv<VEC>(w, m, v, e0, wv, mv, vv);
        if (mark && d == 0) last[row] = target;
    }
}
__global__ void __launch_bounds__(256) k_lazy_mark(const int32_t* __restrict__ uniq_row, const int32_t* __restrict__ uniq_cnt,
                                                   int32_t* __restrict__ last, const int32_t* __restrict__ step_dev, int32_t B,
                                                   int32_t F) {
    const int target = *step_dev - 1;
    const int64_t total = (int64_t)F * B;
    for (int64_t slot = (int64_t)blockIdx.x * blockDim.x + threadIdx.x; slot < total; slot += (int64_t)gridDim.x * blockDim.x) {
        const RowItem it = row_item<1>(slot, 1, B, uniq_cnt, uniq_row);
        if (!it.live) continue;
        if (last[it.row] < target) last[it.row] = target;
    }
}

extern "C" int cdc_embed_lazy_catchup(const int32_t* uniq_row, const int32_t* uniq_cnt, float* w, float* m, float* v,
                                      int32_t* last, cdc_adam_hp hp, const int32_t* step_dev, double* reg_ring,
                                      int32_t ring_len, int64_t B, int32_t F, int32_t D, void* stream) {
    (void)reg_ring; (void)ring_len;
    CDC_CHECK_ARG(uniq_row && uniq_cnt && w && m && v && last && step_dev && hp.step_scalars && hp.n_scalars > 0, CDC_E_BADARG,
                  "embed_lazy_catchup: null pointer");
    CDC_CHECK_ARG(B > 0 && F > 0 && D > 0, CDC_E_BADARG, "embed_lazy_catchup: bad sizes");
    const bool vec = (D % 4 == 0) && ((((uintptr_t)w | (uintptr_t)m | (uintptr_t)v) & 15) == 0);
    const int64_t total = (int64_t)F * B * (vec ? D / 4 : D);
    int blocks = (int)std::min<int64_t>(cdc_ceil_div(total, 256), 256 * 16);
    CDC_CHECK_ARG(!hp.fast_replay || hp.inv_bc2, CDC_E_BADARG, "embed_lazy_catchup: fast_replay needs the inv_bc2 table");
    const int32_t chunks = vec ? D / 4 : D;
    const int32_t mark = (64 % chunks == 0) ? 1 : 0;
#define CDC_CATCHUP(FASTV, VECV)                                                                                                 \
    hipLaunchKernelGGL((k_lazy_catchup<FASTV, VECV>), dim3(blocks), dim3(256), 0, (hipStream_t)stream, uniq_row, uniq_cnt, w, m, \
                       v, last, hp, step_dev, (int32_t)B, F, D, mark)
    if (hp.fast_replay) { if (vec) CDC_CATCHUP(true, 4); else CDC_CATCHUP(true, 1); }
    else                { if (vec) CDC_CATCHUP(false, 4); else CDC_CATCHUP(false, 1); }
#undef CDC_CATCHUP
    CDC_LAUNCH_CHECK("embed_lazy_catchup");
    if (!mark) {
        int blocks2 = (int)std::min<int64_t>(cdc_ceil_div((int64_t)F * B, 256), 256 * 16);
        hipLaunchKernelGGL(k_lazy_mark, dim3(blocks2), dim3(256), 0, (hipStream_t)stream, uniq_row, uniq_cnt, last, step_dev,
                           (int32_t)B, F);
        CDC_LAUNCH_CHECK("embed_lazy_mark");
    }
    return 0;
}

#define CG_HOT 32
template <bool FAST>
__global__ void __launch_bounds__(256) k_lazy_catchup_gather(const int32_t* __restrict__ uniq_row, const int32_t* __restrict__ uniq_cnt,
                                                             const int32_t* __restrict__ seg_start, const int32_t* __restrict__ perm,
                                                             float* __restrict__ w, float* __restrict__ m, float* __restrict__ v,
                                                             int32_t* __restrict__ last, cdc_adam_hp hp,
                                                             const int32_t* __restrict__ step_dev, float* __restrict__ out,
                                                             __bf16* __restrict__ out_h, int64_t ld_out_h, int32_t B, int32_t F, int32_t D,
                                                             int32_t n_short_blocks, int32_t hot_cap) {
    typedef __bf16 h4_t __attribute__((ext_vector_type(4)));
    const AdamConsts c = make_consts(hp);
    const int target = *step_dev - 1;
    const int chunks = D / 4;
    const int lane = threadIdx.x & 63;
    const int64_t total = (int64_t)F * B * chunks;
    const int64_t ld_out = (int64_t)F * D;
    auto put = [&](int b, int f, int ch, float x0, float x1, float x2, float x3) {
        *reinterpret_cast<float4*>(out + (int64_t)b * ld_out + (int64_t)f * D + ch * 4) = make_float4(x0, x1, x2, x3);
        if (out_h) {
            h4_t h = {(__bf16)x0, (__bf16)x1, (__bf16)x2, (__bf16)x3};
            *reinterpret_cast<h4_t*>(out_h + (int64_t)b * ld_out_h + (int64_t)f * D + ch * 4) = h;
        }
    };
    if ((int)blockIdx.x >= n_short_blocks) {
        extern __shared__ __attribute__((aligned(16))) unsigned char cg_smem[];
        __shared__ int n_hot;
        int32_t* hot_j = reinterpret_cast<int32_t*>(cg_smem);
        float4* stage = reinterpret_cast<float4*>(hot_j + hot_cap);
        const int f = (int)blockIdx.x - n_short_blocks;
        const int cnt = uniq_cnt[f];
        const int32_t* ss = seg_start + (int64_t)f * (B + 1);
        if (threadIdx.x == 0) n_hot = 0;
        __syncthreads();
        for (int j = threadIdx.x; j < cnt; j += blockDim.x)
            if (ss[j + 1] - ss[j] > CG_HOT) {
                const int slot = atomicAdd(&n_hot, 1);
                if (slot < hot_cap) hot_j[slot] = j;
            }
        __syncthreads();
        const int nh = n_hot < hot_cap ? n_hot : hot_cap;
        const int n_item = nh * chunks;
        for (int base = 0; base < n_item; base += blockDim.x) {
            const int i = base + threadIdx.x;
            const bool has = i < n_item;
            const int hs = has ? i / chunks : 0, ch = has ? i % chunks : 0;
            const int64_t row = has ? uniq_row[(int64_t)f * B + hot_j[hs]] : -1;
            const bool real = has && row >= 0;
            int from = real ? last[row] : target;
            const bool act = real && from < target;
            if (!act) from = target;
            const int64_t e0 = real ? row * D + ch * 4 : 0;
            float wv[4] = {0.f, 0.f, 0.f, 0.f}, mv[4] = {0.f, 0.f, 0.f, 0.f}, vv[4] = {1.f, 1.f, 1.f, 1.f};
            if (real) { const float4 a4 = *reinterpret_cast<const float4*>(w + e0); wv[0] = a4.x; wv[1] = a4.y; wv[2] = a4.z; wv[3] = a4.w; }
            if (act) {
                const float4 b4 = *reinterpret_cast<const float4*>(m + e0), c4 = *reinterpret_cast<const float4*>(v + e0);
                mv[0] = b4.x; mv[1] = b4.y; mv[2] = b4.z; mv[3] = b4.w;
                vv[0] = c4.x; vv[1] = c4.y; vv[2] = c4.z; vv[3] = c4.w;
            }
            adam_replay_wave<FAST, 4>(wv, mv, vv, from, target, c, hp);
            if (act) {
                *reinterpret_cast<float4*>(w + e0) = make_float4(wv[0], wv[1], wv[2], wv[3]);
                *reinterpret_cast<float4*>(m + e0) = make_float4(mv[0], mv[1], mv[2], mv[3]);
                *reinterpret_cast<float4*>(v + e0) = make_float4(vv[0], vv[1], vv[2], vv[3]);
                if (ch == 0) last[row] = target;
            }
            if (has) stage[i] = make_float4(wv[0], wv[1], wv[2], wv[3]);
        }
        __syncthreads();
        for (int hs = 0; hs < nh; ++hs) {
            const int j = hot_j[hs];
            const int p0 = ss[j], n = ss[j + 1] - p0;
            for (int q = threadIdx.x; q < n * chunks; q += blockDim.x) {
                const int b = perm[(int64_t)f * B + p0 + q / chunks], ch = q % chunks;
                const float4 x = stage[hs * chunks + ch];
                put(b, f, ch, x.x, x.y, x.z, x.w);
            }
        }
        return;
    }
    for (int64_t base = (int64_t)blockIdx.x * blockDim.x; base < total; base += (int64_t)n_short_blocks * blockDim.x) {
        const int64_t i = base + threadIdx.x;
        bool has = i < total;
        int ch = 0, f = 0, j = 0, from = target;
        int64_t row = -1;
        int p0 = 0, n = 0;
        if (has) {
            ch = (int)(i % chunks);
            const int64_t slot = i / chunks;
            f = (int)(slot / B);
            j = (int)(slot - (int64_t)f * B);
            has = j < uniq_cnt[f];
        }
        if (has) {
            row = uniq_row[(int64_t)f * B + j];
            p0 = seg_start[(int64_t)f * (B + 1) + j];
            n = seg_start[(int64_t)f * (B + 1) + j + 1] - p0;
            has = n <= CG_HOT;
        }
        const bool real = has && row >= 0;
        if (real) from = last[row];
        const bool act = real && from < target;
        if (!act) from = target;
        if (!__any(has)) continue;
        const int64_t e0 = real ? row * D + ch * 4 : 0;
        float wv[4] = {0.f, 0.f, 0.f, 0.f}, mv[4] = {0.f, 0.f, 0.f, 0.f}, vv[4] = {1.f, 1.f, 1.f, 1.f};
        if (real) {
            const float4 a4 = *reinterpret_cast<const float4*>(w + e0);
            wv[0] = a4.x; wv[1] = a4.y; wv[2] = a4.z; wv[3] = a4.w;
        }
        if (act) {
            const float4 b4 = *reinterpret_cast<const float4*>(m + e0), c4 = *reinterpret_cast<const float4*>(v + e0);
            mv[0] = b4.x; mv[1] = b4.y; mv[2] = b4.z; mv[3] = b4.w;
            vv[0] = c4.x; vv[1] = c4.y; vv[2] = c4.z; vv[3] = c4.w;
        }
        int bq[4] = {0, 0, 0, 0};
        const bool inline_seg = has && n <= 4;
        if (inline_seg) {
#pragma unroll
            for (int q = 0; q < 4; ++q)
                if (q < n) bq[q] = perm[(int64_t)f * B + p0 + q];
        }
        adam_replay_wave<FAST, 4>(wv, mv, vv, from, target, c, hp);
        if (act) {
            *reinterpret_cast<float4*>(w + e0) = make_float4(wv[0], wv[1], wv[2], wv[3]);
            *reinterpret_cast<float4*>(m + e0) = make_float4(mv[0], mv[1], mv[2], mv[3]);
            *reinterpret_cast<float4*>(v + e0) = make_float4(vv[0], vv[1], vv[2], vv[3]);
            if (ch == 0) last[row] = target;
        }
        if (inline_seg) {
#pragma unroll
            for (int q = 0; q < 4; ++q)
                if (q < n) put(bq[q], f, ch, wv[0], wv[1], wv[2], wv[3]);
        }
        unsigned long long todo = __ballot(has && n > 4 && ch == 0);
        while (todo) {
            const int L = __builtin_amdgcn_readfirstlane(__ffsll((long long)todo) - 1);
            todo &= todo - 1;
            const int sf = __builtin_amdgcn_readlane(f, L), sp0 = __builtin_amdgcn_readlane(p0, L), sn = __builtin_amdgcn_readlane(n, L);
            const int items = sn * chunks;
            const int pc = lane % chunks, ppl = lane / chunks, pstep = 64 / chunks;
            const float x0 = __shfl(wv[0], L + pc, 64), x1 = __shfl(wv[1], L + pc, 64);
            const float x2 = __shfl(wv[2], L + pc, 64), x3 = __shfl(wv[3], L + pc, 64);
            (void)items;
            for (int pb = ppl; pb < sn; pb += 8 * pstep) {
// ... 365 lines not shown
```

causal-domain-clustering-for-multi-domain-recommendation_amd/optim.py:

```python
import collections
import ctypes as C
import math

import os

import torch

from . import _lib as L


def step_scalar_table(lr, beta1, beta2, n=4096, truncate=False):
    rows = [(0.0, 1.0)]
    for t in range(1, n):
        rows.append((lr / (1.0 - beta1 ** t), math.sqrt(1.0 - beta2 ** t)))
    tab = torch.tensor(rows, dtype=torch.float64).to(torch.float32)
    if truncate:
        same = (tab == tab[-1]).all(dim=1)
        first = int(torch.nonzero(~same).max().item()) + 1 if bool((~same).any()) else 0
        tab = tab[:first + 1].contiguous()
    return tab


def _f32(v):
    return float(torch.tensor(v, dtype=torch.float64).to(torch.float32))


ReplayConstants = collections.namedtuple("ReplayConstants", "inv_bc2 replay_tab k1 k2 ik1 ik2 k1_lo k2_lo")


def replay_constants(tab, lerp_w, omb2, eps, wd, l2_table):
    inv_bc2 = (1.0 / tab[:, 1].double()).to(torch.float32).contiguous()
    k1 = k2 = ik1 = ik2 = k1_lo = k2_lo = 0.0
    replay_tab = None
    c = float(torch.tensor(2.0 * _f32(l2_table) + wd, dtype=torch.float64).to(torch.float32))
    if c > 0.0:
        k1r, k2r = _f32(lerp_w * c), _f32(omb2 * c * c)
        if k1r > 0.0 and k2r > 0.0:
            ik1, ik2 = _f32(1.0 / k1r), _f32(1.0 / k2r)
            K1, K2 = 1.0 / ik1, 1.0 / ik2
            k1, k2 = _f32(K1), _f32(K2)
            k1_lo, k2_lo = _f32(K1 - k1), _f32(K2 - k2)
            t64 = tab.double()
            A = t64[:, 0] * K1 * t64[:, 1] / math.sqrt(K2)
            E = eps * t64[:, 1] / math.sqrt(K2)
            A[0] = A[1]
            rt = torch.stack([-1.0 / A, -E / A], dim=1)
            replay_tab = rt.to(torch.float32).contiguous()
    return ReplayConstants(inv_bc2, replay_tab, k1, k2, ik1, ik2, k1_lo, k2_lo)


class FusedAdam:
    def __init__(self, model, lr=1e-3, betas=(0.9, 0.99), eps=1e-8, weight_decay=1e-8, table_mode="dense", frozen=(),
                 fast_replay=True, flush_every=64):
        assert table_mode in ("dense", "lazy")
        self.model = model
        self.frozen = {id(p) for p in frozen}
        self.lib = L.load()
        self.lr, self.betas, self.eps, self.weight_decay = lr, betas, eps, weight_decay
        self.table_mode = table_mode
        self.table = model.embedding.embedding_dict.weight
        dev = self.table.device
        if dev.type != "cuda":
            raise L.HipExtensionError("FusedAdam needs the model on a GPU; there is no CPU fallback")
        self.device = dev
        self.step_dev = torch.zeros(1, dtype=torch.int32, device=dev)
        tab = step_scalar_table(lr, betas[0], betas[1], n=65536, truncate=True)
        self.scalars = tab.to(dev).contiguous()
        self.fast_replay = bool(fast_replay) and table_mode == "lazy"
        self.flush_every = int(flush_every) if table_mode == "lazy" else 0
        self.reg_sum = torch.zeros(2, dtype=torch.float64, device=dev)
        self.table_reg = torch.zeros((), dtype=torch.float64, device=dev)
        self.table_reg_ready = False
        f32 = lambda v: float(torch.tensor(v, dtype=torch.float64).to(torch.float32))
        self._lerp_w = f32(1.0 - betas[0])
        self._beta2 = f32(betas[1])
        self._omb2 = f32(1.0 - betas[1])
        self._eps = f32(eps)
        self._wd = f32(weight_decay)
        l2_of = {}
        for p, l1, l2 in model.regularized_parameters():
            if l1:
                raise NotImplementedError("l1 regularisation is never enabled by the reference's models")
            l2_of[id(p)] = l2_of.get(id(p), 0.0) + l2
        self._l2_of = l2_of
        self.l2_table = l2_of.get(id(self.table), 0.0)
        rc = replay_constants(tab, self._lerp_w, self._omb2, self._eps, self._wd, self.l2_table)
        self._k1 = self._k2 = self._ik1 = self._ik2 = self._k1_lo = self._k2_lo = 0.0
        self.replay_tab = None
        if self.fast_replay and rc.replay_tab is not None:
            self._k1, self._k2, self._ik1, self._ik2, self._k1_lo, self._k2_lo = rc.k1, rc.k2, rc.ik1, rc.ik2, rc.k1_lo, rc.k2_lo
            self.replay_tab = rc.replay_tab.to(dev).contiguous()
        self.inv_bc2 = rc.inv_bc2.to(dev).contiguous()
        self.state = {}
        self.table_m = torch.zeros_like(self.table.data)
        self.table_v = torch.zeros_like(self.table.data)
        self.table_last = torch.zeros(self.table.shape[0], dtype=torch.int32, device=dev) if table_mode == "lazy" else None
        self.own_mod, self.own_rem = 0, 0
        self._dense_args = None
        self._dense_sig = None
        self._ws = {}
        total_dense = sum(p.numel() + 4 for p in model.parameters() if p is not self.table)
        self.grad_arena = torch.zeros(total_dense, dtype=torch.float32, device=dev)
        self.grad_scale = 1.0

    def _hp(self):
        hp = L.AdamHP()
        hp.lerp_w, hp.beta2, hp.one_minus_beta2, hp.eps = self._lerp_w, self._beta2, self._omb2, self._eps
        hp.weight_decay = self._wd
        hp.l2_twice = 2.0 * float(torch.tensor(self.l2_table, dtype=torch.float64).to(torch.float32))
        hp.step_scalars = self.scalars.data_ptr()
        hp.n_scalars = self.scalars.shape[0]
        hp.fast_replay = 1 if self.fast_replay else 0
        hp.inv_bc2 = self.inv_bc2.data_ptr()
        hp.replay_tab = None if self.replay_tab is None else self.replay_tab.data_ptr()
        hp.k1, hp.k2 = self._k1, self._k2
        hp.ik1, hp.ik2, hp.k1_lo, hp.k2_lo = self._ik1, self._ik2, self._k1_lo, self._k2_lo
        return hp

    def _stream(self):
        return C.c_void_p(torch.cuda.current_stream().cuda_stream)

    def _workspace(self, B, F, D, tag=""):
        key = (B, F, D, tag)
        ws = self._ws.get(key)
        if ws is None:
            dev = self.device
            ws = {"uniq": torch.empty((F, B), dtype=torch.int32, device=dev),
                  "seg": torch.empty((F, B + 1), dtype=torch.int32, device=dev),
                  "perm": torch.empty((F, B), dtype=torch.int32, device=dev),
                  "cnt": torch.zeros((F,), dtype=torch.int32, device=dev),
                  "scratch": torch.empty((2 * F * B,), dtype=torch.int64, device=dev) if B > 1024 else None,
                  "rowgrad": torch.empty((F * B * D,), dtype=torch.float32, device=dev),
                  "side": torch.empty((F * B * 3 * D,), dtype=torch.float32, device=dev) if self.table_mode == "dense" else None}
            self._ws[key] = ws
        return ws

    def begin_step(self):
        s = self._stream()
        L.launch("cdc_begin_step", self.lib.cdc_begin_step, (self.step_dev.data_ptr(), self.reg_sum.data_ptr(), 2), s)

    def sort_rows(self, idx, B, F, D, tag="", runs=0):
        ws = self._workspace(B, F, D, tag)
        if runs > 0:
            if ws.get("merge") is None:
                ws["merge"] = torch.empty((F * B,), dtype=torch.int64, device=self.device)
            L.launch("cdc_embed_merge_dedupe", self.lib.cdc_embed_merge_dedupe,
                     (idx.data_ptr(), ws["uniq"].data_ptr(), ws["seg"].data_ptr(), ws["perm"].data_ptr(), ws["cnt"].data_ptr(),
                      ws["merge"].data_ptr(), B, F, runs), self._stream())
            return ws
        L.launch("cdc_embed_sort_dedupe", self.lib.cdc_embed_sort_dedupe,
                 (idx.data_ptr(), ws["uniq"].data_ptr(), ws["seg"].data_ptr(), ws["perm"].data_ptr(), ws["cnt"].data_ptr(),
                  None if ws["scratch"] is None else ws["scratch"].data_ptr(), B, F), self._stream())
        return ws

    def table_index(self, ids, offsets, idx, B, F, err=None):
        L.launch("cdc_embed_index", self.lib.cdc_embed_index,
                 (ids.data_ptr(), offsets.data_ptr(), idx.data_ptr(), None if err is None else err.data_ptr(), B, F,
                  self.table.shape[0]), self._stream())

    def flush_slice(self, background_waves=0):
        if self.table_mode != "lazy" or self.flush_every <= 1:
            return
        nb = 24.0 * self.table.numel() / self.flush_every / max(self.own_mod, 1)
        if background_waves > 0:
            L.launch("cdc_embed_lazy_flush(slice)", self.lib.cdc_embed_lazy_flush_bg,
                     (self.table.data_ptr(), self.table_m.data_ptr(), self.table_v.data_ptr(), self.table_last.data_ptr(),
                      self.table.shape[0], self.table.shape[1], self._hp(), self.step_dev.data_ptr(), -1, self.flush_every,
                      self.own_mod, self.own_rem, int(background_waves)), self._stream(), nbytes=nb)
            return
        L.launch("cdc_embed_lazy_flush(slice)", self.lib.cdc_embed_lazy_flush,
                 (self.table.data_ptr(), self.table_m.data_ptr(), self.table_v.data_ptr(), self.table_last.data_ptr(),
                  self.table.shape[0], self.table.shape[1], self._hp(), self.step_dev.data_ptr(), -1, self.flush_every,
                  self.own_mod, self.own_rem), self._stream(), nbytes=nb)

    def catchup(self, B, F, D, tag=""):
        assert self.table_mode == "lazy"
        ws = self._workspace(B, F, D, tag)
        L.launch("cdc_embed_lazy_catchup", self.lib.cdc_embed_lazy_catchup,
                 (ws["uniq"].data_ptr(), ws["cnt"].data_ptr(), self.table.data_ptr(), self.table_m.data_ptr(),
                  self.table_v.data_ptr(), self.table_last.data_ptr(), self._hp(), self.step_dev.data_ptr(), None, 0, B, F, D), self._stream())

    def catchup_gather(self, B, F, D, tag, out_ptr, out_h, ld_out_h):
        assert self.table_mode == "lazy"
        ws = self._workspace(B, F, D, tag)
        L.launch("cdc_embed_lazy_catchup_gather", self.lib.cdc_embed_lazy_catchup_gather,
                 (ws["uniq"].data_ptr(), ws["cnt"].data_ptr(), ws["seg"].data_ptr(), ws["perm"].data_ptr(), self.table.data_ptr(),
                  self.table_m.data_ptr(), self.table_v.data_ptr(), self.table_last.data_ptr(), self._hp(), self.step_dev.data_ptr(),
                  out_ptr, out_h, ld_out_h, B, F, D), self._stream(), nbytes=float(B) * F * (D * 4 + 4 + D * 4))

    def begin_step_sort(self, ids, offsets, B, F, D, tag="", err=None, begin=True):
        ws = self._workspace(B, F, D, tag)
        L.launch("cdc_embed_sort_dedupe", self.lib.cdc_embed_sort_dedupe_ids,
                 (ids.data_ptr(), offsets.data_ptr(), self.table.shape[0], self.step_dev.data_ptr() if begin else None,
                  self.reg_sum.data_ptr() if begin else None, 2 if begin else 0,
                  None if err is None else err.data_ptr(),
                  ws["uniq"].data_ptr(), ws["seg"].data_ptr(), ws["perm"].data_ptr(), ws["cnt"].data_ptr(),
                  None if ws["scratch"] is None else ws["scratch"].data_ptr(), B, F), self._stream())
        return ws

    def table_step(self, idx, d_out, B, F, D, tag="", short_segments=False):
        s = self._stream()
        hp = self._hp()
        w, m, v = self.table.data_ptr(), self.table_m.data_ptr(), self.table_v.data_ptr()
        if self.table_mode == "dense":
            ws = self.sort_rows(idx, B, F, D)
            self._segment_sum(ws, d_out, B, F, D, s)
            L.launch("cdc_embed_adam_touched", self.lib.cdc_embed_adam_touched,
                     (ws["rowgrad"].data_ptr(), ws["uniq"].data_ptr(), ws["cnt"].data_ptr(),
                      w, m, v, ws["side"].data_ptr(), hp, self.step_dev.data_ptr(), B, F, D), s)
            L.launch("cdc_embed_adam_dense_pass", self.lib.cdc_embed_adam_dense_pass,
                     (w, m, v, self.table.numel(), hp, self.step_dev.data_ptr(), self.reg_sum.data_ptr() + 8), s,
                     nbytes=24.0 * self.table.numel())
            L.launch("cdc_embed_adam_patch", self.lib.cdc_embed_adam_patch,
                     (ws["side"].data_ptr(), ws["uniq"].data_ptr(), ws["cnt"].data_ptr(), w, m, v, B, F, D), s)
        else:
            ws = self._workspace(B, F, D, tag)
            L.launch("cdc_embed_segsum_lazy_update", self.lib.cdc_embed_segsum_lazy_update,
                     (d_out.data_ptr(), ws["seg"].data_ptr(), ws["perm"].data_ptr(), ws["cnt"].data_ptr(), ws["uniq"].data_ptr(),
                      w, m, v, self.table_last.data_ptr(), hp, self.step_dev.data_ptr(), B, F, D, 1 if short_segments else 0), s)

    def _segment_sum(self, ws, d_out, B, F, D, s, short=False):
        if short:
            L.launch("cdc_embed_segment_sum", self.lib.cdc_embed_segment_sum_direct,
                     (d_out.data_ptr(), ws["seg"].data_ptr(), ws["perm"].data_ptr(), ws["cnt"].data_ptr(), ws["uniq"].data_ptr(),
                      ws["rowgrad"].data_ptr(), B, F, D), s)
            return
        L.launch("cdc_embed_segment_sum", self.lib.cdc_embed_segment_sum,
                 (d_out.data_ptr(), ws["seg"].data_ptr(), ws["perm"].data_ptr(), ws["cnt"].data_ptr(), None,
                  ws["rowgrad"].data_ptr(), B, F, D), s)

    def flush_table(self):
        if self.table_mode != "lazy":
            return
        L.launch("cdc_embed_lazy_flush", self.lib.cdc_embed_lazy_flush,
                 (self.table.data_ptr(), self.table_m.data_ptr(), self.table_v.data_ptr(), self.table_last.data_ptr(),
                  self.table.shape[0], self.table.shape[1], self._hp(), self.step_dev.data_ptr(), 0, 0, self.own_mod, self.own_rem),
                 self._stream(), nbytes=24.0 * self.table.numel())

    def dense_step(self, param_grads, param_refs, slabs=None):
        self._dense_prepare(param_grads, param_refs, slabs, False)
        s = self._stream()
        if getattr(self, "_dense_table", None) is not None:
            hdr, tab, wg_t, wg_c, n_wg = self._dense_table
            L.launch("cdc_adam_multi", self.lib.cdc_adam_multi_table, (C.byref(hdr), tab.data_ptr(), wg_t.data_ptr(), wg_c.data_ptr(), n_wg), s)
        for a in self._dense_args:
            L.launch("cdc_adam_multi", self.lib.cdc_adam_multi, (C.byref(a),), s)

    def rows_and_dense_step(self, idx, d_out, B, F, D, param_grads, param_refs, slabs=None, tag="", short_segments=False):
        if self.table_mode != "lazy":
            raise RuntimeError("rows_and_dense_step: lazy table only")
        self._dense_prepare(param_grads, param_refs, slabs, True)
        if self._dense_table is None:
            return self.table_step(idx, d_out, B, F, D, tag=tag, short_segments=short_segments)
        hdr, tab, wg_t, wg_c, n_wg = self._dense_table
        ws = self._workspace(B, F, D, tag)
        L.launch("cdc_embed_segsum_lazy_update_dense", self.lib.cdc_embed_segsum_lazy_update_dense,
                 (d_out.data_ptr(), ws["seg"].data_ptr(), ws["perm"].data_ptr(), ws["cnt"].data_ptr(), ws["uniq"].data_ptr(),
                  self.table.data_ptr(), self.table_m.data_ptr(), self.table_v.data_ptr(), self.table_last.data_ptr(), self._hp(),
                  self.step_dev.data_ptr(), B, F, D, 1 if short_segments else 0, C.byref(hdr), tab.data_ptr(), wg_t.data_ptr(), wg_c.data_ptr(),
                  n_wg), self._stream())

    def _dense_prepare(self, param_grads, param_refs, slabs, table_form):
        slabs = slabs or {}
        sig = (tuple((k, g.data_ptr(), slabs.get(g.data_ptr())) for k, g in param_grads.items()), bool(table_form))
        cache = self.__dict__.setdefault("_dense_cache", {})
        hit = cache.get(sig)
        if hit is not None:
            self._dense_args, self._dense_table = hit
            self._dense_sig = sig
        if self._dense_sig != sig:
            items = []
            for k, g in param_grads.items():
                p = param_refs[k]
                if p is self.table or id(p) in self.frozen:
                    continue
                st = self.state.get(k)
                if st is None:
                    st = (torch.zeros_like(p.data), torch.zeros_like(p.data))
                    self.state[k] = st
                items.append((p, g, st))
            self._dense_table = None
            if len(items) > L.MAX_TENSORS or (table_form and items):
                tab = (L.AdamTensor * len(items))()
                wg_t, wg_c = [], []
                for i, item in enumerate(items):
                    self._adam_tensor(tab[i], item, slabs)
                    nck = -(-item[0].numel() // L.ADAM_CHUNK)
                    wg_t += [i] * nck
                    wg_c += list(range(nck))
                hdr = self._adam_header(0, seed_reg=True)
                dev_tab = torch.frombuffer(bytearray(bytes(tab)), dtype=torch.uint8).to(self.device)
                self._dense_table = (hdr, dev_tab, torch.tensor(wg_t, dtype=torch.int32, device=self.device),
                                     torch.tensor(wg_c, dtype=torch.int32, device=self.device), len(wg_t))
                items = []
            args = []
            for c0 in range(0, len(items), L.MAX_TENSORS):
                chunk = items[c0:c0 + L.MAX_TENSORS]
                a = self._adam_header(len(chunk), seed_reg=c0 == 0)
                for i, item in enumerate(chunk):
                    self._adam_tensor(a.t[i], item, slabs)
                args.append(a)
            self._dense_args, self._dense_sig = args, sig
            cache[sig] = (args, self._dense_table)

    def _adam_header(self, n_tensors, seed_reg):
        a = L.AdamArgs()
        a.n_tensors = n_tensors
        a.lerp_w, a.beta2, a.one_minus_beta2, a.eps, a.weight_decay = self._lerp_w, self._beta2, self._omb2, self._eps, self._wd
        a.step_scalars, a.n_scalars = self.scalars.data_ptr(), self.scalars.shape[0]
        a.grad_scale = self.grad_scale
        a.step_dev = self.step_dev.data_ptr()
        a.reg_sum = self.reg_sum.data_ptr()
        a.reg_seed = self.table_reg.data_ptr() if (self.table_mode == "lazy" and seed_reg) else 0
        return a

    def _adam_tensor(self, T, item, slabs):
        p, g, st = item
        T.w, T.g, T.m, T.v, T.n = p.data_ptr(), g.data_ptr(), st[0].data_ptr(), st[1].data_ptr(), p.numel()
        T.l2 = float(torch.tensor(self._l2_of.get(id(p), 0.0), dtype=torch.float64).to(torch.float32))
        sl = slabs.get(g.data_ptr())
        T.slabs, T.slab_stride, T.n_slabs = sl if sl is not None else (None, 0, 0)

    def reg_loss(self):
        if self.table_mode == "lazy":
            return self.reg_sum[0]
        return self.reg_sum[0] + self.l2_table * self.reg_sum[1]

    def table_reg_loss(self, owned_only=False):
        self.flush_table()
        w = self.table.data
        if owned_only and self.own_mod > 1:
            w = w[self.own_rem::self.own_mod]
        total = torch.zeros((), dtype=torch.float64, device=self.device)
        step = 1 << 22
        for r0 in range(0, w.shape[0], step):
            total += torch.sum(torch.square(w[r0:r0 + step].double()))
        return self.l2_table * total

    def refresh_table_reg(self, dist=None):
        if self.table_mode != "lazy":
            return self.table_reg
        sharded = dist is not None and self.own_mod > 1
        val = self.table_reg_loss(owned_only=sharded)
        if sharded:
            val = val.reshape(1).clone()
            dist.all_reduce_sum(val)
            val = val[0]
        self.table_reg.copy_(val)
        self.table_reg_ready = True
        return self.table_reg

    def state_dict(self):
        self.flush_table()
        names = {id(p): n for n, p in self.model.named_parameters()}
        st = {names[k]: {"exp_avg": m.clone(), "exp_avg_sq": v.clone()} for k, (m, v) in self.state.items() if k in names}
        st[names[id(self.table)]] = {"exp_avg": self.table_m.clone(), "exp_avg_sq": self.table_v.clone()}
        return {"step": int(self.step_dev.item()), "state": st,
                "hyper": {"lr": self.lr, "betas": self.betas, "eps": self.eps, "weight_decay": self.weight_decay}}

    def load_state_dict(self, sd):
        params = dict(self.model.named_parameters())
        self.step_dev.fill_(int(sd["step"]))
        for n, st in sd["state"].items():
            p = params[n]
            if p is self.table:
                self.table_m.copy_(st["exp_avg"])
                self.table_v.copy_(st["exp_avg_sq"])
            else:
                have = self.state.get(id(p))
                if have is not None and have[0].shape == st["exp_avg"].shape:
                    have[0].copy_(st["exp_avg"])
                    have[1].copy_(st["exp_avg_sq"])
                else:
                    self.state[id(p)] = (st["exp_avg"].to(self.device).clone(), st["exp_avg_sq"].to(self.device).clone())
                    self._dense_sig = None
                    self.__dict__.pop("_dense_cache", None)
        if self.table_last is not None:
            self.table_last.fill_(int(sd["step"]))
        self.table_reg_ready = False
```

causal-domain-clustering-for-multi-domain-recommendation_amd/trainer.py:

```python
import ctypes as C
import os

import torch

from . import _lib as L
from .optim import FusedAdam


def _run_steps(steps):
    def fn():
        st = C.c_void_p(torch.cuda.current_stream().cuda_stream)
        for s_ in steps:
            s_(st)
    return fn


def _merge_pieces(seq):
    merged = []
    for is_comm, fn in seq:
        if merged and not is_comm and not merged[-1][0]:
            merged[-1][1].append(fn)
        else:
            merged.append((is_comm, [fn]))
    return merged


class TrainStep:

    def __init__(self, model, optimizer: FusedAdam, batch_size, mode="multi", use_graph=False, dist=None, sync_bn=True,
                 table_dist=None, shard_slack=1.5, train_mode=True, overlap=True, overlap_waves=2, sort_ahead=True, fuse_gather=False,
                 defer_dw_reduce=None, global_rows=None, cap_rows=None, tower_one_launch=True, rows_dense_one_launch=True):
        self.model, self.opt, self.B, self.mode = model, optimizer, int(batch_size), mode
        self.lib = L.load()
        self.dist = dist
        self.sync_bn = bool(sync_bn)
        self.world = 1 if dist is None else dist.world_size
        self.dp_on = self.world > 1 or bool(getattr(dist, "force", False))
        self.global_B = self.B * self.world if global_rows is None else int(global_rows)
        self._shard_slack = float(shard_slack)
        dev = optimizer.device
        self.device = dev
        self.train_mode = bool(train_mode)
        self._overlap_ok, self._overlap_waves = bool(overlap), int(overlap_waves)
        self._rows_dense_one = bool(rows_dense_one_launch) and not self.dp_on
        self.tower_one_launch = bool(tower_one_launch)
        self._defer_dw = (not self.dp_on) if defer_dw_reduce is None else (bool(defer_dw_reduce) and not self.dp_on)
        assert mode in ("multi", "single", "mean", "star", "single_group")
        self.holder = self._build_plan()
        self.plan = self.holder.plan
        self.emb = self.holder.emb_op
        self.out = self.holder.outputs[0]
        self.y = torch.zeros(self.B, dtype=torch.int16, device=dev)
        self.group = torch.zeros(self.B, dtype=torch.int64, device=dev) if mode == "multi" else None
        if mode == "single_group":
            self.group_in = self.holder.inputs[1]
        if mode == "star":
            self.group = self.holder.inputs[1]
            self.order = self.holder.extra_outputs[0]
            self.y_perm = torch.zeros(self.B, dtype=torch.int16, device=dev)
        self.loss = torch.zeros(1, dtype=torch.float32, device=dev)
        self.field_dims_dev = torch.tensor([int(d) for d in model.feature_dims], dtype=torch.int32, device=dev)
        self.alias = torch.zeros(1, dtype=torch.int32, device=dev)
        self.reg = self.opt.reg_sum[0] if self.opt.table_mode == "lazy" else torch.zeros((), dtype=torch.float64, device=dev)
        self.use_graph = use_graph
        self.graph = None
        self._stage_graphs = {}
        self._step_graphs = {}
        self._one_graph_ok = None
        self._dp_seq = None
        self._warm = 0
        self._reg_checked = False
        if table_dist is None:
            table_dist = "sharded" if optimizer.table_mode == "lazy" else "replicated"
        assert table_dist in ("sharded", "replicated")
        self.table_dist = table_dist if self.dp_on else "replicated"
        if self.dp_on and self.table_dist == "replicated":
            F, D = self.emb.F, self.emb.D
            self.idx_all = torch.empty((self.global_B, F), dtype=torch.int32, device=dev)
            self.dE_all = torch.empty((self.global_B, F * D), dtype=torch.float32, device=dev)
            self._loss_behind_arena()
        if self.dp_on and self.table_dist == "sharded":
            if optimizer.table_mode != "lazy":
                raise ValueError("the row-sharded table needs table_mode='lazy'")
            F, D, N = self.emb.F, self.emb.D, self.world
            Bc = self.B if cap_rows is None else int(cap_rows)
            assert Bc >= self.B
            cap = min(Bc, int(-(-Bc // N) * float(shard_slack)) + 16)
            if N * cap > L.SORT_MAX_ROWS:
                raise ValueError(f"world {N} x list capacity {cap} exceeds the per-field sort limit {L.SORT_MAX_ROWS}")
            self.cap, self.Bv = cap, N * cap
            z = dict(device=dev)
            self.send_ids = torch.full((N, cap, F), -1, dtype=torch.int32, **z)
            self.recv_ids = torch.full((N, cap, F), -1, dtype=torch.int32, **z)
            self.recv_ids_alt = torch.full((N, cap, F), -1, dtype=torch.int32, **z)
            self.slot_of = torch.zeros((F, self.B), dtype=torch.int32, **z)
            self.overflow = torch.zeros(1, dtype=torch.int32, **z)
            self.rows_send = torch.zeros((N, cap, F * D), dtype=torch.float32, **z)
            self.rows_recv = torch.zeros((N, cap, F * D), dtype=torch.float32, **z)
            self.grads_send = torch.zeros((N, cap, F * D), dtype=torch.float32, **z)
            self.grads_recv = torch.zeros((N, cap, F * D), dtype=torch.float32, **z)
            self.zero_offsets = torch.zeros(F, dtype=torch.int32, **z)
            optimizer.own_mod, optimizer.own_rem = N, dist.rank
            self._loss_behind_arena()
        lazy_one = optimizer.table_mode == "lazy" and not self.dp_on
        D = self.emb.D
        self._fuse_gather_ok = lazy_one and bool(fuse_gather) and D % 4 == 0 and 64 % (D // 4) == 0
        self._ahead_ok = lazy_one and self._overlap_ok and bool(sort_ahead) and not self._fuse_gather_ok
        self._ahead_dp_ok = (self.dp_on and self.table_dist == "sharded" and bool(sort_ahead) and
                             (self.world > 1 or sort_ahead == "force"))
        self._stage_begins = lazy_one or self._ahead_dp_ok
        self._parity, self._sorted_for = 0, None
        self._graphs, self._dp_seqs = {}, {}
        if self._ahead_ok or self._ahead_dp_ok:
            self.ids_next = torch.zeros_like(self.emb.ids)

    def _loss_behind_arena(self):
        used = max(self.plan._arena_used, 1)
        assert self.opt.grad_arena.numel() > used
        self.arena_and_loss = self.opt.grad_arena[:used + 1]
        self.loss = self.opt.grad_arena[used:used + 1]

    def _build_plan(self):
        model, opt = self.model, self.opt
        B = self.B
        dev = opt.device
        from .functional import PlanHolder
        from . import plan as P

        def build():
            plan = P.Plan(dev, B, precision=model.precision, training=self.train_mode,
                          dropout=float(getattr(model, "dropout_p", 0.0)) if self.train_mode else 0.0,
                          seed=int(getattr(model, "seed", 0)), step_dev=opt.step_dev, grad_arena=opt.grad_arena,
                          dist=self.dist if self.sync_bn else None, defer_dw_reduce=self._defer_dw)
            emb = model.embedding.describe(plan)
            outs, ins, extra = model.describe(plan, emb, grouped=True) if self.mode == "star" else model.describe(plan, emb)
            plan.finalize(outs)
            return PlanHolder(plan, [emb.ids] + ins, outs, emb_op=emb, extra_outputs=extra)

        was = model.training
        model.train(self.train_mode)
        try:
            return model._cache().get(model, ("train_step", id(opt), self.train_mode, self.mode == "star",
                                               bool(self.sync_bn and self.dp_on), bool(self.dp_on), self._defer_dw), B, build)
        finally:
            model.train(was)

    def _find_head(self):
        from . import plan as P
        out = self.out
        for op in self.plan.ops:
            if isinstance(op, (P.TowerHead, P.TowerChain)) and op.sigmoid and op.out.key == out.key:
                if len(op.bwd_args) == 1 and op.M == self.B:
                    self._head_op = op
                    return op.bwd_args[0]
                return None
        for op in self.plan.ops:
            if not isinstance(op, P.RowDot) or not op.sigmoid or op.row_offsets is not None or len(op.groups) != out.cols:
                continue
            if all(g["out"].key == out.slice(i, i + 1).key for i, g in enumerate(op.groups)):
                return op.bwd_args[0] if len(op.bwd_args) == 1 and op.M == self.B else None
        return None

    def _head_lookup(self):
        head = self.__dict__.get("_head", False)
        if head is False:
            self._head_op = None
            head = self._head = self._find_head()
            self._fuse_bce = head is not None and self.mode in ("multi", "single", "single_group")
            if self._fuse_bce:
                self._bce_partial = torch.zeros(L.MAX_GROUPS * L.ROWDOT_PARTS, dtype=torch.float64, device=self.device)
            from . import plan as P
            self._tower_both = (self._head_op if self._fuse_bce and self.tower_one_launch and not self.dp_on and
                                isinstance(self._head_op, P.TowerChain) and self.plan.dist is None else None)
        return head

    def _towers_one_launch(self, on):
        self._head_lookup()
        if self._tower_both is not None:
            self._tower_both.one_launch = bool(on)

    def _bce(self):
        og = self.out.grad
        head = self._head_lookup()
        if head is not None:
            if self._fuse_bce:
                head.bce_group = None if self.group is None else self.group.data_ptr()
                head.bce_y_i16, head.bce_y_f32 = self.y.data_ptr(), None
                head.bce_loss = self.loss.data_ptr()
                if hasattr(type(head), "bce_partial"):
                    head.bce_partial = self._bce_partial.data_ptr()
                head.bce_inv_count = 1.0 / self.global_B
                return
            head.bce_y_i16 = head.bce_y_f32 = None
        if self.mode == "mean":
            L.launch("cdc_bce_mean_fwd_bwd", self.lib.cdc_bce_mean_fwd_bwd,
                     (self.out.ptr, self.out.ld, self.y.data_ptr(), None, self.loss.data_ptr(), og.ptr, og.ld, self.B, self.out.cols,
                      1.0 / self.global_B), C.c_void_p(torch.cuda.current_stream().cuda_stream))
            return
        y, group = self.y, self.group
        if self.mode == "star":
            torch.index_select(self.y, 0, self.order.long(), out=self.y_perm)
            y, group = self.y_perm, None
        L.launch("cdc_bce_fwd_bwd", self.lib.cdc_bce_fwd_bwd,
                 (self.out.ptr, self.out.ld, None if group is None else group.data_ptr(), y.data_ptr(), None,
                  self.loss.data_ptr(), og.ptr, og.ld, self.B, self.out.cols, 1.0 / self.global_B),
                 C.c_void_p(torch.cuda.current_stream().cuda_stream))

    def _reg(self):
        if self.opt.table_mode != "lazy":
            torch.add(self.opt.reg_sum[0], self.opt.reg_sum[1], alpha=self.opt.l2_table, out=self.reg)

    def refresh_table_reg(self):
        sharded = self.dp_on and self.table_dist == "sharded"
        return self.opt.refresh_table_reg(self.dist if sharded else None)

    def _launch(self, have, prefetch, p):
        opt, plan, emb = self.opt, self.plan, self.emb
        B, F, D = self.B, emb.F, emb.D
        main = torch.cuda.current_stream()
        st = C.c_void_p(main.cuda_stream)
        self._towers_one_launch(True)
        try:
            if opt.table_mode != "lazy":
                opt.begin_step()
                plan.forward()
                self._bce()
                plan.backward()
                opt.table_step(emb.idx, emb.out.grad.root, B, F, D)
                opt.dense_step(plan.param_grads, plan._param_refs, plan.grad_slabs)
                self._reg()
                return
            cur, nxt = f"a{p}", f"a{1 - p}"
            bg, fused = self._overlap_ok, self._fuse_gather_ok
            side = self._side_stream() if bg else main
            if bg:
                side.wait_stream(main)
            with torch.cuda.stream(side):
                if not have:
                    opt.begin_step_sort(emb.ids, emb.offsets, B, F, D, tag=cur, err=emb.err if fused else None, begin=False)
                if fused:
                    oh, ldh = plan.shadow_view(emb.out) if (plan.use_g2 and plan.has_shadow(emb.out)) else (None, 0)
                    opt.catchup_gather(B, F, D, cur, emb.out.ptr, oh, ldh)
                else:
                    opt.catchup(B, F, D, cur)
                if bg:
                    rows_ready = torch.cuda.Event()
                    rows_ready.record(side)
                opt.flush_slice(background_waves=self._overlap_waves if bg else 0)
                if prefetch:
                    opt.begin_step_sort(self.ids_next, emb.offsets, B, F, D, tag=nxt, begin=False)
            nws = plan.n_wshadow_steps
            for fn in plan.fwd_steps[:nws]:
                fn(st)
            if bg:
                main.wait_event(rows_ready)
            for fn in plan.fwd_steps[nws:]:
                if not (fused and fn is emb.fwd_step):
                    fn(st)
            self._bce()
            plan.backward()
            if self._rows_dense_one:
                if bg:
                    main.wait_stream(side)
                opt.rows_and_dense_step(emb.idx, emb.out.grad.root, B, F, D, plan.param_grads, plan._param_refs, plan.grad_slabs, tag=cur)
            else:
                opt.dense_step(plan.param_grads, plan._param_refs, plan.grad_slabs)
                if bg:
                    main.wait_stream(side)
                opt.table_step(emb.idx, emb.out.grad.root, B, F, D, tag=cur)
            self._reg()
        finally:
            self._towers_one_launch(False)

    def _lookahead(self, X, nx):
        key = (X.data_ptr(), X._version) if torch.is_tensor(X) else None
        have = self._sorted_for is not None and self._sorted_for[:2] == key
        p = self._parity
        if nx is not None:
            self._parity = 1 - p
            self._sorted_for = (nx.data_ptr(), nx._version, nx)
        else:
            self._sorted_for = None
        return have, nx is not None, p

    def _drop_graphs(self):
        self._step_graphs.clear()
        self._stage_graphs.clear()
        self._graphs.clear()
        self.graph = None

    def _side_stream(self):
        if getattr(self, "_side", None) is None:
            self._side = torch.cuda.Stream(device=self.device)
        return self._side

    def _dp_sequence(self):
        opt, plan, emb, dp = self.opt, self.plan, self.emb, self.dist
        F, D = emb.F, emb.D

        def stage0():
            opt.begin_step()
            opt.table_index(emb.ids, emb.offsets, emb.idx, self.B, F)

        def catchup():
            if opt.table_mode == "lazy":
                opt.sort_rows(self.idx_all, self.global_B, F, D)
                opt.catchup(self.global_B, F, D)
                opt.flush_slice()

        def exchange():
            dp.all_reduce_sum(self.arena_and_loss)
            dp.all_gather_rows(self.dE_all, emb.out.grad.root)

        def update():
            opt.table_step(self.idx_all, self.dE_all, self.global_B, F, D)
            opt.dense_step(plan.param_grads, plan._param_refs, plan.grad_slabs)
            self._reg()

        seq = [(False, stage0), (True, lambda: dp.all_gather_rows(self.idx_all, emb.idx)), (False, catchup)]
        seq += [(is_comm, _run_steps(steps)) for is_comm, steps in plan.segments(plan.fwd_steps)]
        seq.append((False, self._bce))
        seq += [(is_comm, _run_steps(steps)) for is_comm, steps in plan.segments(plan.bwd_steps)]
        seq += [(True, exchange), (False, update)]
        return _merge_pieces(seq)

    def _dp_sequence_sharded(self, ahead=False, have=False, prefetch=False, p=0):
        opt, plan, emb, dp = self.opt, self.plan, self.emb, self.dist
        B, F, D, N, cap, Bv = self.B, emb.F, emb.D, self.world, self.cap, self.Bv
        lib = self.lib
        bufs = (self.recv_ids, self.recv_ids_alt)
        recv_cur, recv_nxt = bufs[p], bufs[1 - p]
        side_ok = self._overlap_ok and (not self.use_graph or (getattr(dp, "capturable", False) and self._one_graph_ok is not False))

        def st():
            return C.c_void_p(torch.cuda.current_stream().cuda_stream)

        def sort_bucket(ids, begin):
            ws = opt.begin_step_sort(ids, emb.offsets, B, F, D, "local", err=emb.err, begin=begin)
            L.launch("cdc_shard_bucket", lib.cdc_shard_bucket,
                     (ws["uniq"].data_ptr(), ws["cnt"].data_ptr(), self.send_ids.data_ptr(), self.slot_of.data_ptr(),
                      self.overflow.data_ptr(), B, F, N, cap), st())

        def stage0():
            sort_bucket(emb.ids, begin=not ahead)

        def stage0_next():
            sort_bucket(self.ids_next, begin=False)

        def serve():
            opt.sort_rows(recv_cur, Bv, F, D, "owner", runs=N)
            opt.catchup(Bv, F, D, "owner")
            if side_ok:
                main, side = torch.cuda.current_stream(), self._side_stream()
                side.wait_stream(main)
                with torch.cuda.stream(side):
                    opt.flush_slice(background_waves=self._overlap_waves)
            L.launch("cdc_embed_gather_fwd(owner)", lib.cdc_embed_gather_fwd,
                     (recv_cur.data_ptr(), self.zero_offsets.data_ptr(), opt.table.data_ptr(), self.rows_send.data_ptr(),
                      None, None, Bv, F, D, opt.table.shape[0]), st())

        emb_shadow = plan.shadow_convert_step(emb.out) if (plan.use_g2 and plan.has_shadow(emb.out)) else None

        def expand():
            ws = opt._workspace(B, F, D, "local")
            L.launch("cdc_shard_expand", lib.cdc_shard_expand,
                     (self.rows_recv.data_ptr(), ws["uniq"].data_ptr(), ws["cnt"].data_ptr(), ws["seg"].data_ptr(),
                      ws["perm"].data_ptr(), self.slot_of.data_ptr(), emb.out.ptr, B, F, D, N, cap), st())
            if emb_shadow is not None:
                emb_shadow(st())

        def pack():
            ws = opt._workspace(B, F, D, "local")
            opt._segment_sum(ws, emb.out.grad.root, B, F, D, st())
            L.launch("cdc_shard_pack", lib.cdc_shard_pack,
                     (ws["rowgrad"].data_ptr(), ws["uniq"].data_ptr(), ws["cnt"].data_ptr(), self.slot_of.data_ptr(),
                      self.grads_send.data_ptr(), B, F, D, N, cap), st())

        pending = {}

        def exchange_rows_start():
            pending["grads"] = dp.all_to_all_start(self.grads_recv, self.grads_send)

        def exchange_finish():
            dp.wait(pending.pop("grads", None))
            dp.all_reduce_sum(self.arena_and_loss)
            if prefetch:
                self._ids_pending = dp.all_to_all_start(recv_nxt, self.send_ids)

        def ids_await():
            dp.wait(self.__dict__.pop("_ids_pending", None))

        def update():
            if side_ok:
                torch.cuda.current_stream().wait_stream(self._side_stream())
            if side_ok:
                opt.rows_and_dense_step(recv_cur, self.grads_recv, Bv, F, D, plan.param_grads, plan._param_refs, plan.grad_slabs, tag="owner",
                                        short_segments=True)
                self._reg()
                return
            opt.table_step(recv_cur, self.grads_recv, Bv, F, D, "owner", short_segments=True)
            opt.flush_slice()
            opt.dense_step(plan.param_grads, plan._param_refs, plan.grad_slabs)
            self._reg()

        def stage0_next_side():
            main, side = torch.cuda.current_stream(), self._side_stream()
            side.wait_stream(main)
            with torch.cuda.stream(side):
                sort_bucket(self.ids_next, begin=False)

        def join_side():
            torch.cuda.current_stream().wait_stream(self._side_stream())

        if have:
            seq = [(True, ids_await), (False, serve)]
        else:
            seq = [(False, stage0), (True, lambda: dp.all_to_all(recv_cur, self.send_ids)), (False, serve)]
        seq += [(True, lambda: dp.all_to_all(self.rows_recv, self.rows_send)), (False, expand)]
        fwd = [s_ for s_ in plan.fwd_steps if s_ is not emb.fwd_step]
        seq += [(is_comm, _run_steps(steps)) for is_comm, steps in plan.segments(fwd)]
        seq.append((False, self._bce))
        late = set(id(s_) for s_ in plan.deferred_dw_steps)
# ... 233 lines not shown
```

include/cdcmdr.h:

```cpp
#ifndef CDCMDR_H
#define CDCMDR_H

#include <stdint.h>

#ifdef __cplusplus
extern "C" {
#endif

#define CDC_ABI_VERSION 1

#define CDC_E_BADARG   (-1)
#define CDC_E_TOOBIG   (-2)
#define CDC_E_ALIGN    (-3)

#define CDC_PREC_BF16 0
#define CDC_PREC_F32  1

#define CDC_MAX_GROUPS 32
#define CDC_MAX_TENSORS 48

int cdc_abi_version(void);
const char* cdc_last_error(void);


int cdc_embed_gather_fwd(const int32_t* ids, const int32_t* offsets, const float* table,
                         float* out, int32_t* idx_out, int32_t* err_flag,
                         int64_t B, int32_t F, int32_t D, int64_t R, void* stream);

int cdc_embed_gather_fwd_h(const int32_t* ids, const int32_t* offsets, const float* table,
                           float* out, void* out_h, int64_t ld_out_h, int32_t* idx_out, int32_t* err_flag,
                           int64_t B, int32_t F, int32_t D, int64_t R, void* stream);

int cdc_embed_index(const int32_t* ids, const int32_t* offsets, int32_t* idx_out, int32_t* err_flag, int64_t B, int32_t F,
                    int64_t R, void* stream);

#define CDC_SORT_MAX_B 16384
#define CDC_SORT_MAX_ROWS 32768
int cdc_embed_sort_dedupe(const int32_t* idx, int32_t* uniq_row, int32_t* seg_start, int32_t* perm,
                          int32_t* uniq_cnt, uint64_t* scratch, int64_t B, int32_t F, void* stream);
int cdc_embed_sort_dedupe_ids(const int32_t* ids, const int32_t* offsets, int64_t R, int32_t* step_dev, double* accumulators,
                              int32_t n_acc, int32_t* err_flag, int32_t* uniq_row, int32_t* seg_start, int32_t* perm,
                              int32_t* uniq_cnt, uint64_t* scratch, int64_t B, int32_t F, void* stream);

int cdc_embed_segment_sum(const float* d_out, const int32_t* seg_start, const int32_t* perm, const int32_t* uniq_cnt,
                          float* sorted_scratch, float* rowgrad, int64_t B, int32_t F, int32_t D, void* stream);
int cdc_embed_segment_sum_direct(const float* d_out, const int32_t* seg_start, const int32_t* perm, const int32_t* uniq_cnt,
                                 const int32_t* uniq_row, float* rowgrad, int64_t B, int32_t F, int32_t D, void* stream);

int cdc_embed_grad_dense(const float* rowgrad, const int32_t* uniq_row, const int32_t* uniq_cnt, float* grad,
                         int64_t B, int32_t F, int32_t D, int64_t R, void* stream);

typedef struct {
    float lerp_w, beta2, one_minus_beta2, eps, weight_decay, l2_twice;
    const float* step_scalars;
    int32_t n_scalars;
    int32_t fast_replay;
    const float* inv_bc2;
    const float* replay_tab;
    float k1, k2;
    float ik1, ik2, k1_lo, k2_lo;
} cdc_adam_hp;

int cdc_embed_adam_touched(const float* rowgrad, const int32_t* uniq_row, const int32_t* uniq_cnt,
                           const float* w, const float* m, const float* v, float* side,
                           cdc_adam_hp hp, const int32_t* step_dev,
                           int64_t B, int32_t F, int32_t D, void* stream);
int cdc_embed_adam_dense_pass(float* w, float* m, float* v, int64_t n_elems,
                              cdc_adam_hp hp, const int32_t* step_dev, double* reg_sum, void* stream);
int cdc_embed_adam_patch(const float* side, const int32_t* uniq_row, const int32_t* uniq_cnt,
                         float* w, float* m, float* v, int64_t B, int32_t F, int32_t D, void* stream);

int cdc_embed_lazy_catchup(const int32_t* uniq_row, const int32_t* uniq_cnt,
                           float* w, float* m, float* v, int32_t* last,
                           cdc_adam_hp hp, const int32_t* step_dev, double* reg_ring, int32_t ring_len,
                           int64_t B, int32_t F, int32_t D, void* stream);
int cdc_embed_lazy_update(const float* rowgrad, const int32_t* uniq_row, const int32_t* uniq_cnt,
                          float* w, float* m, float* v, int32_t* last,
                          cdc_adam_hp hp, const int32_t* step_dev, double* reg_ring, int32_t ring_len,
                          int64_t B, int32_t F, int32_t D, void* stream);
int cdc_embed_lazy_catchup_gather(const int32_t* uniq_row, const int32_t* uniq_cnt, const int32_t* seg_start, const int32_t* perm,
                                  float* w, float* m, float* v, int32_t* last, cdc_adam_hp hp, const int32_t* step_dev,
                                  float* out, void* out_h, int64_t ld_out_h, int64_t B, int32_t F, int32_t D, void* stream);
int cdc_embed_segsum_lazy_update(const float* d_out, const int32_t* seg_start, const int32_t* perm, const int32_t* uniq_cnt,
                                 const int32_t* uniq_row, float* w, float* m, float* v, int32_t* last, cdc_adam_hp hp,
                                 const int32_t* step_dev, int64_t B, int32_t F, int32_t D, int32_t short_only, void* stream);
int cdc_embed_lazy_flush(float* w, float* m, float* v, int32_t* last, int64_t R, int32_t D,
                         cdc_adam_hp hp, const int32_t* step_dev, int32_t step_bias, int32_t period,
                         int32_t own_mod, int32_t own_rem, void* stream);
int cdc_embed_lazy_flush_bg(float* w, float* m, float* v, int32_t* last, int64_t R, int32_t D,
                            cdc_adam_hp hp, const int32_t* step_dev, int32_t step_bias, int32_t period,
                            int32_t own_mod, int32_t own_rem, int32_t waves_per_simd, void* stream);

int cdc_embed_merge_dedupe(const int32_t* idx, int32_t* uniq_row, int32_t* seg_start, int32_t* perm, int32_t* uniq_cnt,
                           uint64_t* scratch, int64_t B, int32_t F, int32_t n_runs, void* stream);
int cdc_shard_bucket(const int32_t* uniq_row, const int32_t* uniq_cnt, int32_t* send_ids, int32_t* slot_of, int32_t* overflow,
                     int64_t B, int32_t F, int32_t n_rank, int32_t cap, void* stream);
int cdc_shard_expand(const float* rows_recv, const int32_t* uniq_row, const int32_t* uniq_cnt, const int32_t* seg_start,
                     const int32_t* perm, const int32_t* slot_of, float* out, int64_t B, int32_t F, int32_t D,
                     int32_t n_rank, int32_t cap, void* stream);
int cdc_shard_pack(const float* rowgrad, const int32_t* uniq_row, const int32_t* uniq_cnt, const int32_t* slot_of, float* send,
                   int64_t B, int32_t F, int32_t D, int32_t n_rank, int32_t cap, void* stream);

typedef struct {
    const float* x;  int64_t ldx;
    const float* w;  int64_t ldw;
    const float* bias;
    float* y;        int64_t ldy;
    int32_t M, N, K;
    int32_t act_cols;
    double* bn_partial;
    int32_t bn_col0, bn_total_c;
} cdc_lin_group;

typedef struct {
    int32_t n_groups;
    int32_t relu;
    float   drop_p;
    uint64_t seed;
    const int32_t* seed_offset_dev;
    const int32_t* row_offsets;
    cdc_lin_group g[CDC_MAX_GROUPS];
} cdc_lin_fwd_args;

int cdc_glinear_fwd(const cdc_lin_fwd_args* a, int32_t prec, void* stream);

typedef struct {
    const float* dz; int64_t lddz;
    const float* w;  int64_t ldw;
    const float* wt; int64_t ldwt;
    int32_t N;
    int32_t out;
    int32_t wt_bf16;
} cdc_bwdx_seg;
typedef struct {
    float* dx; int64_t lddx;
    const float* mask_y; int64_t ldmask;
    int32_t M, K;
    int32_t mask_cols;
    int32_t accumulate;
} cdc_bwdx_out;
typedef struct {
    int32_t n_out, n_seg;
    float mask_scale;
    const int32_t* row_offsets;
    cdc_bwdx_out o[CDC_MAX_GROUPS];
    cdc_bwdx_seg s[CDC_MAX_GROUPS];
} cdc_lin_bwdx_args;
int cdc_glinear_bwd_x(const cdc_lin_bwdx_args* a, int32_t prec, void* stream);

typedef struct {
    int32_t n;
    int32_t pad_;
    uint64_t bf16_mask;
    struct { const float* src; float* dst; int32_t rows, cols; } t[CDC_MAX_TENSORS];
} cdc_transpose_args;
int cdc_transpose_multi(const cdc_transpose_args* a, void* stream);

#define CDC_G2_MAX_OUT 24
#define CDC_G2_MAX_SEG 32
typedef struct {
    float* y; int64_t ldy;
    void*  yh; int64_t ldyh;
    const float* bias;
    const void* mask; int64_t ldmask;
    double* bn_partial;
    int32_t M, N;
    int32_t act_cols;
    int32_t accumulate;
    int32_t mask_bf16;
    int32_t bn_col0, bn_total_c;
    int32_t stream_id;
} cdc_g2_out;
typedef struct {
    const void* a; int64_t lda;
    const void* b; int64_t ldb;
    int32_t Kr;
    int32_t out;
} cdc_g2_seg;
typedef struct {
    int32_t n_out, n_seg;
    int32_t mode;
    int32_t relu;
    float   drop_p;
    float   mask_scale;
    int32_t tile_cfg;
    int32_t pad_;
    uint64_t seed;
    const int32_t* seed_offset_dev;
    cdc_g2_out o[CDC_G2_MAX_OUT];
    cdc_g2_seg s[CDC_G2_MAX_SEG];
} cdc_g2_args;
int cdc_gemm_bf16_nt(const cdc_g2_args* a, void* stream);

typedef struct {
    int32_t n;
    int32_t pad_;
    struct { const float* src; void* dst_h; int64_t ld_h; void* dst_t; int64_t ld_t; int32_t rows, cols; } t[CDC_MAX_TENSORS];
} cdc_wshadow_args;
int cdc_weight_shadows(const cdc_wshadow_args* a, void* stream);

typedef struct {
    int32_t n;
    int32_t pad_;
    struct { const float* src; int64_t ld_src; void* dst; int64_t ld_dst; int64_t rows; int32_t cols; int32_t pad_; } t[CDC_MAX_GROUPS];
} cdc_shadow_args;
int cdc_shadow_bf16(const cdc_shadow_args* a, void* stream);

typedef struct {
    const float* dz; int64_t lddz;
    const float* x;  int64_t ldx;
    float* dw; int64_t lddw;
    float* db;
    int32_t M, N, K;
    int32_t accumulate;
    const void* dzh; int64_t lddzh;
    const void* xh;  int64_t ldxh;
} cdc_bwdw_group;
typedef struct {
    int32_t n_groups;
    int32_t split_k;
    float* workspace;
    const int32_t* row_offsets;
    int32_t defer_reduce;
    int32_t pad_;
    cdc_bwdw_group g[CDC_MAX_GROUPS];
} cdc_lin_bwdw_args;
int cdc_glinear_bwd_w(const cdc_lin_bwdw_args* a, int32_t prec, void* stream);
int cdc_glinear_bwd_w_pair(const cdc_lin_bwdw_args* wide, const cdc_lin_bwdw_args* narrow, const cdc_lin_bwdw_args* tabs_dev, void* stream);
int cdc_glinear_bwd_w_pair_reduce(const cdc_lin_bwdw_args* wide, const cdc_lin_bwdw_args* narrow, const cdc_lin_bwdw_args* tabs_dev,
                                  void* stream);

#define CDC_MAX_GATES 16
#define CDC_MAX_SEL   16
typedef struct {
    int32_t n_gates, n_expert, H;
    int64_t B;
    const float* experts; int64_t ld_exp;
    struct {
// ... 300 lines not shown
    float* out; int64_t ld_out;
    const float* d_out; int64_t ld_dout;
    const float* wide_x; int64_t ld_wide;
    const float* wide_w; const float* wide_bias;
    float* wide_out; int64_t ld_wide_out;
    float* wide_dx; int64_t ld_wide_dx;
    float* wide_dw; float* wide_dbias;
    int32_t wide_K, accumulate_wide_dx;
    const float* addend[2]; int64_t ld_addend[2];
    float* d_addend[2]; int64_t ld_d_addend[2];
    int32_t accumulate_d_addend[2];
    float* workspace;
    const int64_t* bce_group;
    const int16_t* bce_y_i16;
    const float* bce_y_f32;
    float* bce_loss;
    double* bce_partial;
    float bce_inv_count;
    int32_t pad2_;
    cdc_head_tower t[CDC_HEAD_MAX_TOWERS];
} cdc_head_args;
int cdc_head_fwd(const cdc_head_args* a, void* stream);
int cdc_head_bwd(const cdc_head_args* a, void* stream);
int64_t cdc_head_workspace_floats(const cdc_head_args* a);

#define CDC_TOWER_MAX 4
#define CDC_TOWER_ROWS 128
#define CDC_TOWER_ERR_TIMEOUT 0x40000000
typedef struct {
    const void* wh; int64_t ldwh;
    const void* wt; int64_t ldwt;
    const float* bias;
    float* z; int64_t ldz;
    void* dzh; int64_t lddzh;
    const float* gamma; const float* beta;
    float* running_mean; float* running_var;
    int64_t* num_batches_tracked;
    float* save_mean; float* save_invstd;
    float* dgamma; float* dbeta;
} cdc_tower_layer;
typedef struct {
    const void* xh; int64_t ldxh;
    float* dx; int64_t lddx;
    int32_t accumulate_dx, pad_;
    cdc_tower_layer l1, l2;
    void* a1h; int64_t lda1h;
    float* a2; int64_t lda2;
    const float* wo; const float* bo;
    float* dwo; float* dbo;
    float* dy2; int64_t lddy2;
    float* dy1; int64_t lddy1;
} cdc_tower_desc;
typedef struct {
    int32_t n_tower, H0, H1, H2;
    int64_t M;
    int32_t relu, sigmoid;
    float drop_p, eps, momentum;
    int32_t pad_;
    uint64_t seed1, seed2;
    const int32_t* seed_offset_dev;
    float* out; int64_t ld_out;
    const float* d_out; int64_t ld_dout;
    const float* wide_x; int64_t ld_wide;
    const float* wide_w; const float* wide_bias;
    float* wide_dx; int64_t ld_wide_dx;
    float* wide_dw; float* wide_dbias;
    int32_t wide_K, accumulate_wide_dx;
    const int64_t* bce_group;
    const int16_t* bce_y_i16;
    const float* bce_y_f32;
    float* bce_loss;
    float bce_inv_count;
    int32_t pad2_;
    void* workspace;
    int32_t* err;
    double* exchange[4];
    cdc_tower_desc t[CDC_TOWER_MAX];
} cdc_tower_args;
int64_t cdc_tower_workspace_bytes(const cdc_tower_args* a);
int cdc_tower_fwd(const cdc_tower_args* a, void* stream);
int cdc_tower_bwd(const cdc_tower_args* a, void* stream);
int cdc_tower_step(const cdc_tower_args* a, void* stream);
int cdc_tower_dp(const cdc_tower_args* a, int32_t phase, void* stream);

int cdc_bce_fwd_bwd(const float* p, int64_t ldp, const int64_t* group, const int16_t* y_i16,
                    const float* y_f32, float* loss, float* dp, int64_t lddp,
                    int64_t B, int32_t n_col, float inv_count, void* stream);
int cdc_bce_mean_fwd_bwd(const float* p, int64_t ldp, const int16_t* y_i16, const float* y_f32, float* loss, float* dp,
                         int64_t lddp, int64_t B, int32_t n_col, float inv_count, void* stream);

int cdc_fm_fwd(const float* e, int64_t lde, float* out, int64_t ldo, int64_t B, int32_t F, int32_t D, void* stream);
int cdc_fm_bwd(const float* e, int64_t lde, const float* dout, int64_t ldd, float* de, int64_t ldde, int64_t B, int32_t F,
               int32_t D, int32_t accumulate, void* stream);

int cdc_group_select_fwd(const float* feas, int64_t ldf, const int64_t* group, float* out, int64_t ldo, int64_t B,
                         int32_t n_group, int32_t H, void* stream);
int cdc_group_select_bwd(const float* dout, int64_t ldd, const int64_t* group, float* dfeas, int64_t ldf, int64_t B,
                         int32_t n_group, int32_t H, int32_t accumulate, void* stream);

int cdc_sigmoid_gate_fwd(const float* a, int64_t lda, const float* p, int64_t ldp, float* out, int64_t ldo, int64_t rows,
                         int32_t cols, float beta, float alpha, float eps, void* stream);
int cdc_sigmoid_gate_bwd(const float* a, int64_t lda, const float* p, int64_t ldp, const float* dout, int64_t lddo, float* da,
                         int64_t ldda, int32_t acc_a, float* dp, int64_t lddp, int32_t acc_p, int64_t rows, int32_t cols,
                         float beta, float alpha, float eps, void* stream);

int cdc_cross_fwd(const float* x0, int64_t ld0, const float* xl, int64_t ldl, const float* w, const float* b,
                  float* out, int64_t ldo, float* xw_save, int64_t B, int32_t E, void* stream);
int cdc_cross_bwd(const float* d_out, int64_t ldo, const float* x0, int64_t ld0, const float* xl, int64_t ldl,
                  const float* w, const float* xw_save, float* d_x0_acc, int64_t ld_dx0, float* d_xl, int64_t ld_dxl,
                  float* dw, float* db, float* workspace, int64_t B, int32_t E, void* stream);

int cdc_tanh_fwd(const float* x, int64_t ldx, float* y, int64_t ldy, int64_t rows, int32_t cols, void* stream);
int cdc_tanh_bwd(const float* dy, int64_t lddy, const float* y, int64_t ldy, float* dx, int64_t lddx,
                 int64_t rows, int32_t cols, int32_t accumulate, void* stream);
int cdc_cross_combine_fwd(const float* x0, int64_t ld0, const float* u, int64_t ldu, const float* b1, const float* b2,
                          const float* r, int64_t ldr, float* out, int64_t ldo, int64_t rows, int32_t period, int32_t n_rep,
                          void* stream);
int cdc_cross_combine_bwd(const float* d_out, int64_t lddo, const float* x0, int64_t ld0, const float* u, int64_t ldu,
                          const float* b1, float* d_u, int64_t lddu, float* d_x0_acc, int64_t lddx0, float* d_r, int64_t lddr,
                          int32_t accumulate_r, float* db1, int32_t accumulate_b1, float* db2, int32_t accumulate_b2,
                          float* workspace, int64_t rows, int32_t period, int32_t n_rep, void* stream);
int cdc_add_out(const float* a, int64_t lda, const float* b, int64_t ldb, float* out, int64_t ldo,
                int64_t rows, int32_t cols, void* stream);
int cdc_copy_or_add(float* dst, int64_t ldd, const float* src, int64_t lds, int64_t rows, int32_t cols,
                    int32_t accumulate, void* stream);

typedef struct {
    float* w; const float* g; float* m; float* v;
    int64_t n;
    float l2;
    int32_t n_slabs;
    const float* slabs;
    int64_t slab_stride;
} cdc_adam_tensor;
typedef struct {
    int32_t n_tensors;
    float lerp_w, beta2, one_minus_beta2, eps, weight_decay;
    const float* step_scalars; int32_t n_scalars;
    float grad_scale;
    const int32_t* step_dev;
    double* reg_sum;
    const double* reg_seed;
    cdc_adam_tensor t[CDC_MAX_TENSORS];
} cdc_adam_args;
int cdc_adam_multi(const cdc_adam_args* a, void* stream);
#define CDC_ADAM_CHUNK 4096
int cdc_adam_multi_table(const cdc_adam_args* a, const cdc_adam_tensor* tensors_dev, const int32_t* wg_tensor_dev,
                         const int32_t* wg_chunk_dev, int32_t n_workgroups, void* stream);
int cdc_embed_segsum_lazy_update_dense(const float* d_out, const int32_t* seg_start, const int32_t* perm, const int32_t* uniq_cnt,
                                       const int32_t* uniq_row, float* w, float* m, float* v, int32_t* last, cdc_adam_hp hp,
                                       const int32_t* step_dev, int64_t B, int32_t F, int32_t D, int32_t short_only,
                                       const cdc_adam_args* dense, const cdc_adam_tensor* tensors_dev, const int32_t* wg_tensor_dev,
                                       const int32_t* wg_chunk_dev, int32_t n_dense_workgroups, void* stream);

typedef struct {
    int32_t n;
    int32_t op;
    int64_t size;
    const float* s;
    float* ds;
    int32_t accumulate_ds;
    int32_t pad_;
    const float* a[CDC_MAX_GROUPS];
    float* out[CDC_MAX_GROUPS];
    float* da[CDC_MAX_GROUPS];
} cdc_star_fuse_args;
int cdc_star_fuse_fwd(const cdc_star_fuse_args* a, void* stream);
int cdc_star_fuse_bwd(const cdc_star_fuse_args* a, void* stream);

int cdc_sum_slices(const float* in, int64_t ld_in, float* out, int64_t ld_out, int64_t rows, int32_t cols,
                   int32_t n_slices, int32_t accumulate, void* stream);

int cdc_step_increment(int32_t* step_dev, void* stream);
int cdc_begin_step(int32_t* step_dev, double* accumulators, int32_t n_acc, void* stream);
int cdc_stage_batch(const int32_t* ids, const int16_t* y, const int64_t* group, int32_t* ids_dst, int16_t* y_dst,
                    int64_t* group_dst, int64_t B, int32_t F, const int32_t* field_dims, int32_t* alias_flag, void* stream);
int cdc_stage_batch_next(const int32_t* ids, const int16_t* y, const int64_t* group, int32_t* ids_dst, int16_t* y_dst,
                         int64_t* group_dst, int64_t B, int32_t F, const int32_t* next_ids, int32_t* next_dst,
                         int32_t* step_dev, double* accumulators, int32_t n_acc, const int32_t* field_dims, int32_t* alias_flag,
                         void* stream);
int cdc_fill_f32(float* p, float value, int64_t n, void* stream);
int cdc_fill_f64(double* p, double value, int64_t n, void* stream);
int cdc_add_inplace(float* dst, int64_t ld_dst, const float* src, int64_t ld_src, int64_t rows, int32_t cols, void* stream);
typedef struct {
    float* dst; int64_t ld_dst;
    int64_t rows; int32_t cols;
    int32_t n;
    int32_t accumulate;
    const float* src[CDC_MAX_GROUPS];
    int64_t ld_src[CDC_MAX_GROUPS];
} cdc_add_n_args;
int cdc_add_n(const cdc_add_n_args* a, void* stream);
int cdc_mul_bcast(const float* a, const float* b, float* out, int64_t na, int64_t nb, void* stream);
int cdc_mul_bcast_bwd(const float* d_out, const float* a, const float* b, float* da, float* db,
                      int64_t na, int64_t nb, void* stream);
int cdc_group_partition(const int64_t* group, int32_t* row_offsets, int32_t* order,
                        int64_t B, int32_t n_group, void* stream);
int cdc_rows_permute(const float* in, int64_t ld_in, const int32_t* order, float* out, int64_t ld_out,
                     int64_t B, int32_t C, int32_t inverse, void* stream);

int cdc_attn_fwd(const float* qkv, int64_t ld, float* out, int64_t ldo, float* probs, int64_t B, int32_t F, int32_t A, int32_t H,
                 float drop_p, uint64_t seed, const int32_t* seed_offset_dev, void* stream);
int cdc_attn_bwd(const float* qkv, int64_t ld, const float* probs, const float* dout, int64_t lddo, float* dqkv, int64_t lddq,
                 int64_t B, int32_t F, int32_t A, int32_t H, float drop_p, uint64_t seed, const int32_t* seed_offset_dev,
                 void* stream);
int cdc_add_relu_fwd(const float* a, int64_t lda, const float* b, int64_t ldb, float* out, int64_t ldo, int64_t rows, int32_t cols,
                     void* stream);
int cdc_add_relu_bwd(const float* out, int64_t ldo, const float* dout, int64_t lddo, float* da, int64_t ldda, int32_t acc_a,
                     float* db, int64_t lddb, int32_t acc_b, int64_t rows, int32_t cols, void* stream);

int64_t cdc_eval_workspace_bytes(int64_t n, int32_t n_domain);
int cdc_eval_metrics(const float* pred, const int16_t* label, const int32_t* domain, int64_t ld_domain, int64_t n,
                     int32_t n_domain, double* out, int64_t* counts, int32_t* err_flag, void* workspace,
                     int64_t workspace_bytes, void* stream);

int64_t cdc_eval_gauc_workspace_bytes(int64_t n, int32_t n_domain, int64_t n_user);
int cdc_eval_gauc(const float* pred, const int16_t* label, const int32_t* user, int64_t ld_user, int64_t n_user,
                  const int32_t* domain, int64_t ld_domain, int32_t n_domain, const double* user_weight, int64_t n,
                  double* out, int64_t* counts, int32_t* err_flag, void* workspace, int64_t workspace_bytes, void* stream);

int64_t cdc_eval_auc_delong_workspace_bytes(int64_t n, int32_t n_domain, int32_t paired);
int cdc_eval_auc_delong(const float* pred_a, const float* pred_b, const int16_t* label, const int32_t* domain, int64_t ld_domain,
                        int64_t n, int32_t n_domain, double* out, int64_t* counts, int32_t* err_flag, void* workspace,
                        int64_t workspace_bytes, void* stream);

int64_t cdc_eval_loss_ci_workspace_bytes(int64_t n, int32_t n_domain, int32_t paired);
int cdc_eval_loss_ci(const float* pred_a, const float* pred_b, const int16_t* label, const int32_t* domain, int64_t ld_domain,
                     int64_t n, int32_t n_domain, double* out, int64_t* counts, int32_t* err_flag, void* workspace,
                     int64_t workspace_bytes, void* stream);

int64_t cdc_eval_gauc_ci_workspace_bytes(int64_t n, int32_t n_domain, int64_t n_user, int32_t paired);
int cdc_eval_gauc_ci(const float* pred_a, const float* pred_b, const int16_t* label, const int32_t* user, int64_t ld_user,
                     int64_t n_user, const int32_t* domain, int64_t ld_domain, int32_t n_domain, const double* user_weight,
                     int64_t n, double* out, int64_t* counts, int32_t* err_flag, void* workspace, int64_t workspace_bytes,
                     void* stream);

int64_t cdc_eval_bootstrap_workspace_bytes(int64_t n, int32_t n_domain, int64_t n_cluster, int32_t n_rep, int32_t gauc);
int cdc_eval_bootstrap(const float* pred_a, const float* pred_b, const int16_t* label, const int32_t* cluster, int64_t ld_cluster,
                       int64_t n_cluster, const int32_t* domain, int64_t ld_domain, int32_t n_domain, const double* user_weight,
                       int64_t n, int32_t n_rep, uint64_t seed, int32_t gauc, double* out, int64_t* counts, int32_t* err_flag,
                       void* workspace, int64_t workspace_bytes, void* stream);

int64_t cdc_eval_calibration_workspace_bytes(int64_t n, int32_t n_domain, int32_t n_bins);
int cdc_eval_calibration(const float* pred, const int16_t* label, const int32_t* domain, int64_t ld_domain, int64_t n,
                         int32_t n_domain, int32_t n_bins, double* seg_out, int64_t* seg_counts, double* tab_out,
                         int64_t* tab_counts, float* tab_range, int32_t* err_flag, void* workspace, int64_t workspace_bytes,
                         void* stream);

int64_t cdc_eval_calibration_bootstrap_workspace_bytes(int64_t n, int32_t n_domain, int32_t n_bins, int32_t n_rep, int32_t paired);
int cdc_eval_calibration_bootstrap(const float* pred_a, const float* pred_b, const int16_t* label, const int32_t* cluster,
                                   int64_t ld_cluster, int64_t n_cluster, const int32_t* domain, int64_t ld_domain, int32_t n_domain,
                                   int32_t n_bins, int64_t n, int32_t n_rep, uint64_t seed, double* out, int64_t* counts,
                                   int32_t* err_flag, void* workspace, int64_t workspace_bytes, void* stream);

int64_t cdc_eval_isotonic_max_blocks(int64_t n, int32_t n_domain);
int64_t cdc_eval_isotonic_fit_workspace_bytes(int64_t n, int32_t n_domain);
int cdc_eval_isotonic_fit(const float* pred, const int16_t* label, const int32_t* domain, int64_t ld_domain, int64_t n,
                          int32_t n_domain, int64_t* start, float* x_lo, float* x_hi, int64_t* count, int64_t* positives,
                          double* value, int64_t cap, int64_t* seg_rows, int64_t* seg_positives, int32_t* err_flag,
                          void* workspace, int64_t workspace_bytes, void* stream);

int cdc_eval_isotonic_apply(const float* pred, const int32_t* domain, int64_t ld_domain, int64_t n, int32_t n_domain,
                            const int32_t* seg_of_domain, const int64_t* start, const float* x_lo, const float* x_hi,
                            const double* value, float eps, float* out, int32_t* err_flag, void* stream);

#define CDC_PLATT_PLATT 0
#define CDC_PLATT_TEMPERATURE 1
#define CDC_PLATT_BIAS 2
#define CDC_PLATT_INPUT_PROB 0
#define CDC_PLATT_INPUT_LOGIT 1
#define CDC_PLATT_CONVERGED 1
#define CDC_PLATT_EMPTY 2
#define CDC_PLATT_SLOPE_FIXED 4
int64_t cdc_eval_platt_fit_workspace_bytes(int64_t n, int32_t n_domain);
int cdc_eval_platt_fit(const float* score, const int16_t* label, const int32_t* domain, int64_t ld_domain, int64_t n,
                       int32_t n_domain, int32_t method, int32_t input, double clip, double gtol, int32_t max_iter, double* a,
                       double* b, double* loss_before, double* loss_after, double* grad, int64_t* seg_rows, int64_t* seg_positives,
                       int32_t* iterations, int32_t* status, int32_t* err_flag, void* workspace, int64_t workspace_bytes,
                       void* stream);

int cdc_eval_platt_apply(const float* score, const int32_t* domain, int64_t ld_domain, int64_t n, int32_t n_domain,
                         const int32_t* seg_of_domain, const double* a, const double* b, int32_t input, double clip, float eps,
                         float* out, int32_t* err_flag, void* stream);

int cdc_eval_segments(const float* probs, int64_t ld_probs, const int16_t* label, const int32_t* seg_start, int32_t n_seg,
                      const int32_t* seg_col, double* loss, float* sel_pred, int32_t* seg_of_row, int32_t* err_flag, int64_t rows,
                      int32_t n_cols, void* stream);

#ifdef __cplusplus
}
#endif
#endif
```

Baseline: 13.49 million samples/s.

## Stage touched embedding rows' Adam state in slot order during catchup

The lazy catchup pass now writes each touched row's caught-up w/m/v into a compact per-slot staging buffer. The segment-sum Adam update then reads that state with contiguous per-slot loads instead of gathering it again from the million-row tables. This is meant to cut random-access reads in the update kernel, which sits on the critical path, by moving the gather into the catchup that already runs on the side stream. In exchange it adds a staging buffer of 3*D floats per slot, extra writes during catchup, and new staged kernel variants with alignment requirements.

```diff
diff --git a/causal-domain-clustering-for-multi-domain-recommendation_amd/_lib.py b/causal-domain-clustering-for-multi-domain-recommendation_amd/_lib.py
--- a/causal-domain-clustering-for-multi-domain-recommendation_amd/_lib.py
+++ b/causal-domain-clustering-for-multi-domain-recommendation_amd/_lib.py
@@ -352,6 +352,9 @@
     "cdc_embed_adam_dense_pass": (c_i32, [c_p, c_p, c_p, c_i64, AdamHP, c_p, c_p, c_p]),
     "cdc_embed_adam_patch": (c_i32, [c_p, c_p, c_p, c_p, c_p, c_p, c_i64, c_i32, c_i32, c_p]),
     "cdc_embed_lazy_catchup": (c_i32, [c_p, c_p, c_p, c_p, c_p, c_p, AdamHP, c_p, c_p, c_i32, c_i64, c_i32, c_i32, c_p]),
+    "cdc_embed_lazy_catchup_stage": (c_i32, [c_p, c_p, c_p, c_p, c_p, c_p, c_p, AdamHP, c_p, c_i64, c_i32, c_i32, c_p]),
+    "cdc_embed_segsum_lazy_update_staged": (c_i32, [c_p, c_p, c_p, c_p, c_p, c_p, c_p, c_p, c_p, c_p, AdamHP, c_p, c_i64, c_i32, c_i32, c_i32,
+                                                    c_p]),
     "cdc_embed_lazy_catchup_gather": (c_i32, [c_p, c_p, c_p, c_p, c_p, c_p, c_p, c_p, AdamHP, c_p, c_p, c_p, c_i64, c_i64, c_i32, c_i32, c_p]),
     "cdc_embed_lazy_update": (c_i32, [c_p, c_p, c_p, c_p, c_p, c_p, c_p, AdamHP, c_p, c_p, c_i32, c_i64, c_i32, c_i32, c_p]),
     "cdc_embed_lazy_flush": (c_i32, [c_p, c_p, c_p, c_p, c_i64, c_i32, AdamHP, c_p, c_i32, c_i32, c_i32, c_i32, c_p]),
@@ -447,6 +450,8 @@
     "cdc_adam_multi_table": (c_i32, [C.POINTER(AdamArgs), c_p, c_p, c_p, c_i32, c_p]),
     "cdc_embed_segsum_lazy_update_dense": (c_i32, [c_p, c_p, c_p, c_p, c_p, c_p, c_p, c_p, c_p, AdamHP, c_p, c_i64, c_i32, c_i32, c_i32,
                                                    C.POINTER(AdamArgs), c_p, c_p, c_p, c_i32, c_p]),
+    "cdc_embed_segsum_lazy_update_dense_staged": (c_i32, [c_p, c_p, c_p, c_p, c_p, c_p, c_p, c_p, c_p, c_p, AdamHP, c_p, c_i64, c_i32, c_i32,
+                                                          c_i32, C.POINTER(AdamArgs), c_p, c_p, c_p, c_i32, c_p]),
     "cdc_step_increment": (c_i32, [c_p, c_p]),
     "cdc_begin_step": (c_i32, [c_p, c_p, c_i32, c_p]),
     "cdc_fill_f32": (c_i32, [c_p, c_f, c_i64, c_p]),
diff --git a/causal-domain-clustering-for-multi-domain-recommendation_amd/csrc/embedding.hip b/causal-domain-clustering-for-multi-domain-recommendation_amd/csrc/embedding.hip
--- a/causal-domain-clustering-for-multi-domain-recommendation_amd/csrc/embedding.hip
+++ b/causal-domain-clustering-for-multi-domain-recommendation_amd/csrc/embedding.hip
@@ -582,6 +582,21 @@
     store_wmv<VEC>(w, m, v, e0, wv, mv, vv);
     if (d0 == 0) last[row] = t;
 }
+template <int VEC>
+__device__ __forceinline__ void load_row_state(const float* __restrict__ row_state, int64_t slot, int D, int d0, float (&wv)[VEC],
+                                               float (&mv)[VEC], float (&vv)[VEC]) {
+    const float* rec = row_state + slot * 3 * D + d0;
+    load_wmv<VEC>(rec, rec + D, rec + 2 * D, 0, wv, mv, vv);
+}
+template <int VEC>
+__device__ __forceinline__ void row_adam_step_from(float* w, float* m, float* v, int32_t* last, int64_t row, int D, int d0,
+                                                   const float (&g)[VEC], float (&wv)[VEC], float (&mv)[VEC], float (&vv)[VEC],
+                                                   const AdamConsts& c, float step_size, float bc2s, int32_t t) {
+#pragma unroll
+    for (int q = 0; q < VEC; ++q) adam_elem(wv[q], mv[q], vv[q], g[q], c, step_size, bc2s);
+    store_wmv<VEC>(w, m, v, row * D + d0, wv, mv, vv);
+    if (d0 == 0) last[row] = t;
+}
 
 #define SEG_SPLIT 64
 #define SEG_DIRECT 8
@@ -594,12 +609,21 @@
     float* w; float* m; float* v;
     int32_t* last;
     const int32_t* uniq_row;
+    const float* row_state;
     AdamConsts c;
     float step_size, bc2s;
     int32_t t;
 };
-template <int VEC>
+template <int VEC, bool STAGED = false>
 __device__ __forceinline__ void seg_finish(const SegSink& k, int64_t slot, int D, int d0, const float (&acc)[VEC]) {
+    if (STAGED) {
+        float wv[VEC], mv[VEC], vv[VEC];
+        load_row_state<VEC>(k.row_state, slot, D, d0, wv, mv, vv);
+        const int64_t row = k.uniq_row[slot];
+        if (row < 0) return;
+        row_adam_step_from<VEC>(k.w, k.m, k.v, k.last, row, D, d0, acc, wv, mv, vv, k.c, k.step_size, k.bc2s, k.t);
+        return;
+    }
     if (!k.w) {
         float* dst = k.rowgrad + slot * D + d0;
         if (VEC == 4) *reinterpret_cast<float4*>(dst) = make_float4(acc[0], acc[1 % VEC], acc[2 % VEC], acc[3 % VEC]);
@@ -616,7 +640,7 @@
     return k;
 }
 
-template <int VEC>
+template <int VEC, bool STAGED = false>
 __device__ __forceinline__ void seg_direct_body(int bid, int nblocks, const float* __restrict__ d_out, const int32_t* __restrict__ seg_start,
                                                 const int32_t* __restrict__ perm, const int32_t* __restrict__ uniq_cnt,
                                                 const int32_t* __restrict__ uniq_row, const SegSink& sink,
@@ -626,7 +650,13 @@
     for (int64_t i = (int64_t)bid * blockDim.x + threadIdx.x; i < total; i += (int64_t)nblocks * blockDim.x) {
         const RowItem it = row_item<VEC, false>(i, chunks, B, uniq_cnt, nullptr);
         if (!it.live) continue;
-        if (uniq_row && uniq_row[it.slot] < 0) continue;
+        float wv[VEC], mv[VEC], vv[VEC];
+        int64_t row = 0;
+        if (STAGED) {
+            load_row_state<VEC>(sink.row_state, it.slot, D, it.d, wv, mv, vv);
+            row = sink.uniq_row[it.slot];
+            if (uniq_row && row < 0) continue;
+        } else if (uniq_row && uniq_row[it.slot] < 0) continue;
         const int f = it.f, j = it.j;
         const int32_t* sst = seg_start + (int64_t)f * (B + 1);
         const int32_t* prm = perm + (int64_t)f * B;
@@ -659,7 +689,9 @@
                     for (int e = 0; e < VEC; ++e) acc[e] = __fadd_rn(acc[e], v[q][e]);
                 }
         }
-        seg_finish<VEC>(sink, it.slot, D, it.d, acc);
+        if (STAGED && row < 0) continue;
+        if (STAGED) row_adam_step_from<VEC>(sink.w, sink.m, sink.v, sink.last, row, D, it.d, acc, wv, mv, vv, sink.c, sink.step_size, sink.bc2s, sink.t);
+        else seg_finish<VEC>(sink, it.slot, D, it.d, acc);
     }
 }
 template <int VEC>
@@ -703,7 +735,7 @@
     }
     return acc;
 }
-template <int VEC>
+template <int VEC, bool STAGED = false>
 __device__ __forceinline__ void seg_long_body(int f, int by, const float* __restrict__ d_out, const int32_t* __restrict__ seg_start,
                                               const int32_t* __restrict__ perm, const int32_t* __restrict__ uniq_cnt,
                                               const SegSink& sink, int32_t B, int32_t F, int32_t D, int32_t subs,
@@ -731,7 +763,7 @@
         if (subs <= 1) {
             for (int d = lane; d < D; d += 64) {
                 const float one[1] = {seg_serial_sum(d_out, prm + k0, 0, len, F, D, f, d)};
-                seg_finish<1>(sink, slot, D, d, one);
+                seg_finish<1, STAGED>(sink, slot, D, d, one);
             }
             continue;
         }
@@ -751,7 +783,7 @@
         }
         if (sub == 0) {
             const float one[1] = {acc};
-            seg_finish<1>(sink, slot, D, d, one);
+            seg_finish<1, STAGED>(sink, slot, D, d, one);
         }
     }
     if (!block_rows) return;
@@ -804,13 +836,13 @@
             for (int p2 = 1; p2 < P; ++p2)
 #pragma unroll
                 for (int e = 0; e < VEC; ++e) total[e] = __fadd_rn(total[e], parts[(p2 * chunks + tid) * VEC + e]);
-            seg_finish<VEC>(sink, (int64_t)f * B + j, D, tid * VEC, total);
+            seg_finish<VEC, STAGED>(sink, (int64_t)f * B + j, D, tid * VEC, total);
         }
         __syncthreads();
     }
 }
 
-template <int VEC>
+template <int VEC, bool STAGED = false>
 __global__ void __launch_bounds__(256) k_segment_sum(const float* __restrict__ d_out, const int32_t* __restrict__ seg_start,
                                                      const int32_t* __restrict__ perm, const int32_t* __restrict__ uniq_cnt,
                                                      SegSink sink, cdc_adam_hp hp, const int32_t* __restrict__ step_dev, int32_t B,
@@ -822,12 +854,12 @@
     }
     const int n_long = F * SEG_LONG_BLOCKS;
     if ((int)blockIdx.x < n_long)
-        seg_long_body<VEC>(blockIdx.x / SEG_LONG_BLOCKS, blockIdx.x % SEG_LONG_BLOCKS, d_out, seg_start, perm, uniq_cnt, sink, B, F, D,
-                           subs, SEG_DIRECT);
+        seg_long_body<VEC, STAGED>(blockIdx.x / SEG_LONG_BLOCKS, blockIdx.x % SEG_LONG_BLOCKS, d_out, seg_start, perm, uniq_cnt, sink, B, F, D,
+                                   subs, SEG_DIRECT);
     else
-        seg_direct_body<VEC>(blockIdx.x - n_long, gridDim.x - n_long, d_out, seg_start, perm, uniq_cnt, nullptr, sink, B, F, D, SEG_DIRECT);
-}
-template <int VEC>
+        seg_direct_body<VEC, STAGED>(blockIdx.x - n_long, gridDim.x - n_long, d_out, seg_start, perm, uniq_cnt, nullptr, sink, B, F, D, SEG_DIRECT);
+}
+template <int VEC, bool STAGED = false>
 __global__ void __launch_bounds__(256, 4) k_segment_sum_dense(const float* __restrict__ d_out, const int32_t* __restrict__ seg_start,
                                                            const int32_t* __restrict__ perm, const int32_t* __restrict__ uniq_cnt,
                                                            SegSink sink, cdc_adam_hp hp, const int32_t* __restrict__ step_dev, int32_t B,
@@ -847,12 +879,12 @@
     sink.t = *step_dev;
     step_scalars_at(hp.step_scalars, hp.n_scalars, sink.t, sink.step_size, sink.bc2s);
     if (b < n_long)
-        seg_long_body<VEC>(b / SEG_LONG_BLOCKS, b % SEG_LONG_BLOCKS, d_out, seg_start, perm, uniq_cnt, sink, B, F, D, subs, SEG_DIRECT);
+        seg_long_body<VEC, STAGED>(b / SEG_LONG_BLOCKS, b % SEG_LONG_BLOCKS, d_out, seg_start, perm, uniq_cnt, sink, B, F, D, subs, SEG_DIRECT);
     else
-        seg_direct_body<VEC>(b - n_long - n_dense, (int)gridDim.x - n_long - n_dense, d_out, seg_start, perm, uniq_cnt,
-                             short_only ? sink.uniq_row : nullptr, sink, B, F, D, short_only ? 0 : SEG_DIRECT);
-}
-template <int VEC>
+        seg_direct_body<VEC, STAGED>(b - n_long - n_dense, (int)gridDim.x - n_long - n_dense, d_out, seg_start, perm, uniq_cnt,
+                                     short_only ? sink.uniq_row : nullptr, sink, B, F, D, short_only ? 0 : SEG_DIRECT);
+}
+template <int VEC, bool STAGED = false>
 __global__ void __launch_bounds__(256) k_segment_sum_short_sink(const float* __restrict__ d_out, const int32_t* __restrict__ seg_start,
                                                                 const int32_t* __restrict__ perm, const int32_t* __restrict__ uniq_cnt,
                                                                 SegSink sink, cdc_adam_hp hp, const int32_t* __restrict__ step_dev,
@@ -860,7 +892,7 @@
     sink.c = make_consts(hp);
     sink.t = *step_dev;
     step_scalars_at(hp.step_scalars, hp.n_scalars, sink.t, sink.step_size, sink.bc2s);
-    seg_direct_body<VEC>(blockIdx.x, gridDim.x, d_out, seg_start, perm, uniq_cnt, sink.uniq_row, sink, B, F, D, 0);
+    seg_direct_body<VEC, STAGED>(blockIdx.x, gridDim.x, d_out, seg_start, perm, uniq_cnt, sink.uniq_row, sink, B, F, D, 0);
 }
 
 struct SegGeom {
@@ -939,6 +971,57 @@
     return 0;
 }
 
+static int seg_staged_geometry(const char* who, const float* d_out, const float* row_state, float* w, float* m, float* v, int32_t* last,
+                               const int32_t* uniq_row, int64_t B, int32_t F, int32_t D, SegGeom& g) {
+    if (!row_state) { cdc_set_error("%s: row_state is NULL", who); return CDC_E_BADARG; }
+    if (D % 4 != 0) { cdc_set_error("%s: the staged form needs D %% 4 == 0 (D = %d)", who, D); return CDC_E_BADARG; }
+    g = seg_geometry(d_out, nullptr, w, m, v, last, uniq_row, B, F, D);
+    if (!g.vec || (uintptr_t)row_state % 16 != 0) { cdc_set_error("%s: the staged form needs 16-byte aligned buffers", who); return CDC_E_ALIGN; }
+    g.sink.row_state = row_state;
+    return 0;
+}
+extern "C" int cdc_embed_segsum_lazy_update_staged(const float* d_out, const int32_t* seg_start, const int32_t* perm, const int32_t* uniq_cnt,
+                                                   const int32_t* uniq_row, const float* row_state, float* w, float* m, float* v,
+                                                   int32_t* last, cdc_adam_hp hp, const int32_t* step_dev, int64_t B, int32_t F, int32_t D,
+                                                   int32_t short_only, void* stream) {
+    CDC_CHECK_ARG(d_out && seg_start && perm && uniq_cnt && uniq_row && w && m && v && last && step_dev && hp.step_scalars &&
+                      hp.n_scalars > 0, CDC_E_BADARG, "embed_segsum_lazy_update_staged: null pointer");
+    CDC_CHECK_ARG(B > 0 && F > 0 && D > 0 && B <= CDC_SORT_MAX_ROWS, CDC_E_BADARG, "embed_segsum_lazy_update_staged: bad sizes");
+    SegGeom g;
+    if (const int rc = seg_staged_geometry("embed_segsum_lazy_update_staged", d_out, row_state, w, m, v, last, uniq_row, B, F, D, g)) return rc;
+    hipStream_t st = (hipStream_t)stream;
+    if (short_only) {
+        hipLaunchKernelGGL((k_segment_sum_short_sink<4, true>), dim3(g.direct_blocks), dim3(256), 0, st, d_out, seg_start, perm, uniq_cnt, g.sink, hp, step_dev, (int32_t)B, F, D);
+    } else {
+        const int blocks = g.direct_blocks + F * SEG_LONG_BLOCKS;
+        hipLaunchKernelGGL((k_segment_sum<4, true>), dim3(blocks), dim3(256), 0, st, d_out, seg_start, perm, uniq_cnt, g.sink, hp, step_dev, (int32_t)B, F, D, g.subs);
+    }
+    CDC_LAUNCH_CHECK("embed_segsum_lazy_update_staged");
+    return 0;
+}
+extern "C" int cdc_embed_segsum_lazy_update_dense_staged(const float* d_out, const int32_t* seg_start, const int32_t* perm, const int32_t* uniq_cnt,
+                                                         const int32_t* uniq_row, const float* row_state, float* w, float* m, float* v,
+                                                         int32_t* last, cdc_adam_hp hp, const int32_t* step_dev, int64_t B, int32_t F,
+                                                         int32_t D, int32_t short_only, const cdc_adam_args* dense,
+                                                         const cdc_adam_tensor* tensors_dev, const int32_t* wg_tensor_dev,
+                                                         const int32_t* wg_chunk_dev, int32_t n_dense_workgroups, void* stream) {
+    CDC_CHECK_ARG(d_out && seg_start && perm && uniq_cnt && uniq_row && w && m && v && last && step_dev && hp.step_scalars &&
+                      hp.n_scalars > 0, CDC_E_BADARG, "embed_segsum_lazy_update_dense_staged: null pointer");
+    CDC_CHECK_ARG(B > 0 && F > 0 && D > 0 && B <= CDC_SORT_MAX_ROWS, CDC_E_BADARG, "embed_segsum_lazy_update_dense_staged: bad sizes");
+    CDC_CHECK_ARG(dense && tensors_dev && wg_tensor_dev && wg_chunk_dev && n_dense_workgroups > 0 && n_dense_workgroups < (1 << 24) &&
+                      dense->step_dev && dense->step_scalars && dense->n_scalars > 0, CDC_E_BADARG,
+                  "embed_segsum_lazy_update_dense_staged: the dense parameters' descriptor table (as for cdc_adam_multi_table) is missing");
+    SegGeom g;
+    if (const int rc = seg_staged_geometry("embed_segsum_lazy_update_dense_staged", d_out, row_state, w, m, v, last, uniq_row, B, F, D, g)) return rc;
+    const int blocks = g.direct_blocks + (short_only ? 0 : F * SEG_LONG_BLOCKS) + n_dense_workgroups;
+    const AdamHdr h = {dense->lerp_w, dense->beta2, dense->one_minus_beta2, dense->eps, dense->weight_decay, dense->grad_scale,
+                       dense->step_scalars, dense->n_scalars, dense->step_dev, dense->reg_sum, dense->reg_seed};
+    hipLaunchKernelGGL((k_segment_sum_dense<4, true>), dim3(blocks), dim3(256), 0, (hipStream_t)stream, d_out, seg_start, perm, uniq_cnt, g.sink, hp,
+                       step_dev, (int32_t)B, F, D, g.subs, h, tensors_dev, wg_tensor_dev, wg_chunk_dev, n_dense_workgroups, short_only);
+    CDC_LAUNCH_CHECK("embed_segsum_lazy_update_dense_staged");
+    return 0;
+}
+
 __global__ void __launch_bounds__(256) k_grad_dense(const float* __restrict__ rowgrad, const int32_t* __restrict__ uniq_row,
                                                     const int32_t* __restrict__ uniq_cnt, float* __restrict__ grad,
                                                     int32_t B, int32_t F, int32_t D, int64_t R) {
@@ -1141,6 +1224,80 @@
     else                { if (vec) CDC_CATCHUP(false, 4); else CDC_CATCHUP(false, 1); }
 #undef CDC_CATCHUP
     CDC_LAUNCH_CHECK("embed_lazy_catchup");
+    if (!mark) {
+        int blocks2 = (int)std::min<int64_t>(cdc_ceil_div((int64_t)F * B, 256), 256 * 16);
+        hipLaunchKernelGGL(k_lazy_mark, dim3(blocks2), dim3(256), 0, (hipStream_t)stream, uniq_row, uniq_cnt, last, step_dev,
+                           (int32_t)B, F);
+        CDC_LAUNCH_CHECK("embed_lazy_mark");
+    }
+    return 0;
+}
+
+template <bool FAST>
+__global__ void __launch_bounds__(256) k_lazy_catchup_stage(const int32_t* __restrict__ uniq_row, const int32_t* __restrict__ uniq_cnt,
+                                                            float* __restrict__ w, const float* __restrict__ m, const float* __restrict__ v,
+                                                            int32_t* __restrict__ last, float* __restrict__ row_state, cdc_adam_hp hp,
+                                                            const int32_t* __restrict__ step_dev, int32_t B, int32_t F, int32_t D,
+                                                            int32_t mark) {
+    constexpr int VEC = 4;
+    const AdamConsts c = make_consts(hp);
+    const int target = *step_dev - 1;
+    const int chunks = D / VEC;
+    const int64_t total = (int64_t)F * B * chunks;
+    for (int64_t base = (int64_t)blockIdx.x * blockDim.x; base < total; base += (int64_t)gridDim.x * blockDim.x) {
+        const int64_t i = base + threadIdx.x;
+        bool live = false;
+        int d = 0, from = target;
+        int64_t row = -1, slot = 0;
+        if (i < total) {
+            const RowItem it = row_item<VEC, false>(i, chunks, B, uniq_cnt, nullptr);
+            d = it.d;
+            slot = it.slot;
+            row = uniq_row[slot];
+            live = it.live && row >= 0;
+        }
+        float wv[VEC], mv[VEC], vv[VEC];
+#pragma unroll
+        for (int k = 0; k < VEC; ++k) { wv[k] = 0.f; mv[k] = 0.f; vv[k] = 1.f; }
+        const int64_t e0 = live ? row * D + d : 0;
+        if (live) {
+            from = last[row];
+            load_wmv<VEC>(w, m, v, e0, wv, mv, vv);
+        }
+        const bool act = live && from < target;
+        if (!act) from = target;
+        if (!__any(live)) continue;
+        adam_replay_wave<FAST, VEC>(wv, mv, vv, from, target, c, hp);
+        if (!live) continue;
+        float* rec = row_state + slot * 3 * D + d;
+        store_wmv<VEC>(rec, rec + D, rec + 2 * D, 0, wv, mv, vv);
+        if (!act) continue;
+        *reinterpret_cast<float4*>(w + e0) = make_float4(wv[0], wv[1], wv[2], wv[3]);
+        if (mark && d == 0) last[row] = target;
+    }
+}
+extern "C" int cdc_embed_lazy_catchup_stage(const int32_t* uniq_row, const int32_t* uniq_cnt, float* w, const float* m, const float* v,
+                                            int32_t* last, float* row_state, cdc_adam_hp hp, const int32_t* step_dev, int64_t B, int32_t F,
+                                            int32_t D, void* stream) {
+    CDC_CHECK_ARG(uniq_row && uniq_cnt && w && m && v && last && step_dev && hp.step_scalars && hp.n_scalars > 0, CDC_E_BADARG,
+                  "embed_lazy_catchup_stage: null pointer");
+    CDC_CHECK_ARG(row_state, CDC_E_BADARG, "embed_lazy_catchup_stage: row_state is NULL");
+    CDC_CHECK_ARG(B > 0 && F > 0 && D > 0 && B <= CDC_SORT_MAX_ROWS, CDC_E_BADARG, "embed_lazy_catchup_stage: bad sizes");
+    CDC_CHECK_ARG(D % 4 == 0, CDC_E_BADARG, "embed_lazy_catchup_stage: the staged form needs D %% 4 == 0 (D = %d)", D);
+    CDC_CHECK_ARG((((uintptr_t)w | (uintptr_t)m | (uintptr_t)v | (uintptr_t)row_state) & 15) == 0, CDC_E_ALIGN,
+                  "embed_lazy_catchup_stage: the staged form needs 16-byte aligned buffers");
+    CDC_CHECK_ARG(!hp.fast_replay || hp.inv_bc2, CDC_E_BADARG, "embed_lazy_catchup_stage: fast_replay needs the inv_bc2 table");
+    const int32_t chunks = D / 4;
+    const int64_t total = (int64_t)F * B * chunks;
+    const int blocks = (int)std::min<int64_t>(cdc_ceil_div(total, 256), 256 * 16);
+    const int32_t mark = (64 % chunks == 0) ? 1 : 0;
+    if (hp.fast_replay)
+        hipLaunchKernelGGL((k_lazy_catchup_stage<true>), dim3(blocks), dim3(256), 0, (hipStream_t)stream, uniq_row, uniq_cnt, w, m, v, last,
+                           row_state, hp, step_dev, (int32_t)B, F, D, mark);
+    else
+        hipLaunchKernelGGL((k_lazy_catchup_stage<false>), dim3(blocks), dim3(256), 0, (hipStream_t)stream, uniq_row, uniq_cnt, w, m, v, last,
+                           row_state, hp, step_dev, (int32_t)B, F, D, mark);
+    CDC_LAUNCH_CHECK("embed_lazy_catchup_stage");
     if (!mark) {
         int blocks2 = (int)std::min<int64_t>(cdc_ceil_div((int64_t)F * B, 256), 256 * 16);
         hipLaunchKernelGGL(k_lazy_mark, dim3(blocks2), dim3(256), 0, (hipStream_t)stream, uniq_row, uniq_cnt, last, step_dev,
diff --git a/causal-domain-clustering-for-multi-domain-recommendation_amd/optim.py b/causal-domain-clustering-for-multi-domain-recommendation_amd/optim.py
--- a/causal-domain-clustering-for-multi-domain-recommendation_amd/optim.py
+++ b/causal-domain-clustering-for-multi-domain-recommendation_amd/optim.py
@@ -99,6 +99,7 @@
         self._dense_args = None
         self._dense_sig = None
         self._ws = {}
+        self._row_states = {}
         total_dense = sum(p.numel() + 4 for p in model.parameters() if p is not self.table)
         self.grad_arena = torch.zeros(total_dense, dtype=torch.float32, device=dev)
         self.grad_scale = 1.0
@@ -135,6 +136,17 @@
             self._ws[key] = ws
         return ws
 
+    def _row_state(self, B, F, D):
+        key = (B, F, D)
+        rs = self._row_states.get(key)
+        if rs is None:
+            rs = self._row_states[key] = torch.empty((F * B, 3, D), dtype=torch.float32, device=self.device)
+        return rs
+
+    def can_stage_rows(self, D):
+        return (self.table_mode == "lazy" and D % 4 == 0 and
+                all(t.data_ptr() % 16 == 0 for t in (self.table, self.table_m, self.table_v)))
+
     def begin_step(self):
         s = self._stream()
         L.launch("cdc_begin_step", self.lib.cdc_begin_step, (self.step_dev.data_ptr(), self.reg_sum.data_ptr(), 2), s)
@@ -173,9 +185,15 @@
                   self.table.shape[0], self.table.shape[1], self._hp(), self.step_dev.data_ptr(), -1, self.flush_every,
                   self.own_mod, self.own_rem), self._stream(), nbytes=nb)
 
-    def catchup(self, B, F, D, tag=""):
+    def catchup(self, B, F, D, tag="", stage=False):
         assert self.table_mode == "lazy"
         ws = self._workspace(B, F, D, tag)
+        if stage:
+            L.launch("cdc_embed_lazy_catchup_stage", self.lib.cdc_embed_lazy_catchup_stage,
+                     (ws["uniq"].data_ptr(), ws["cnt"].data_ptr(), self.table.data_ptr(), self.table_m.data_ptr(),
+                      self.table_v.data_ptr(), self.table_last.data_ptr(), self._row_state(B, F, D).data_ptr(), self._hp(),
+                      self.step_dev.data_ptr(), B, F, D), self._stream())
+            return
         L.launch("cdc_embed_lazy_catchup", self.lib.cdc_embed_lazy_catchup,
                  (ws["uniq"].data_ptr(), ws["cnt"].data_ptr(), self.table.data_ptr(), self.table_m.data_ptr(),
                   self.table_v.data_ptr(), self.table_last.data_ptr(), self._hp(), self.step_dev.data_ptr(), None, 0, B, F, D), self._stream())
@@ -198,7 +216,7 @@
                   None if ws["scratch"] is None else ws["scratch"].data_ptr(), B, F), self._stream())
         return ws
 
-    def table_step(self, idx, d_out, B, F, D, tag="", short_segments=False):
+    def table_step(self, idx, d_out, B, F, D, tag="", short_segments=False, staged=False):
         s = self._stream()
         hp = self._hp()
         w, m, v = self.table.data_ptr(), self.table_m.data_ptr(), self.table_v.data_ptr()
@@ -215,6 +233,12 @@
                      (ws["side"].data_ptr(), ws["uniq"].data_ptr(), ws["cnt"].data_ptr(), w, m, v, B, F, D), s)
         else:
             ws = self._workspace(B, F, D, tag)
+            if staged:
+                L.launch("cdc_embed_segsum_lazy_update_staged", self.lib.cdc_embed_segsum_lazy_update_staged,
+                         (d_out.data_ptr(), ws["seg"].data_ptr(), ws["perm"].data_ptr(), ws["cnt"].data_ptr(), ws["uniq"].data_ptr(),
+                          self._row_state(B, F, D).data_ptr(), w, m, v, self.table_last.data_ptr(), hp, self.step_dev.data_ptr(), B, F, D,
+                          1 if short_segments else 0), s)
+                return
             L.launch("cdc_embed_segsum_lazy_update", self.lib.cdc_embed_segsum_lazy_update,
                      (d_out.data_ptr(), ws["seg"].data_ptr(), ws["perm"].data_ptr(), ws["cnt"].data_ptr(), ws["uniq"].data_ptr(),
                       w, m, v, self.table_last.data_ptr(), hp, self.step_dev.data_ptr(), B, F, D, 1 if short_segments else 0), s)
@@ -246,14 +270,21 @@
         for a in self._dense_args:
             L.launch("cdc_adam_multi", self.lib.cdc_adam_multi, (C.byref(a),), s)
 
-    def rows_and_dense_step(self, idx, d_out, B, F, D, param_grads, param_refs, slabs=None, tag="", short_segments=False):
+    def rows_and_dense_step(self, idx, d_out, B, F, D, param_grads, param_refs, slabs=None, tag="", short_segments=False, staged=False):
         if self.table_mode != "lazy":
             raise RuntimeError("rows_and_dense_step: lazy table only")
         self._dense_prepare(param_grads, param_refs, slabs, True)
         if self._dense_table is None:
-            return self.table_step(idx, d_out, B, F, D, tag=tag, short_segments=short_segments)
+            return self.table_step(idx, d_out, B, F, D, tag=tag, short_segments=short_segments, staged=staged)
         hdr, tab, wg_t, wg_c, n_wg = self._dense_table
         ws = self._workspace(B, F, D, tag)
+        if staged:
+            L.launch("cdc_embed_segsum_lazy_update_dense_staged", self.lib.cdc_embed_segsum_lazy_update_dense_staged,
+                     (d_out.data_ptr(), ws["seg"].data_ptr(), ws["perm"].data_ptr(), ws["cnt"].data_ptr(), ws["uniq"].data_ptr(),
+                      self._row_state(B, F, D).data_ptr(), self.table.data_ptr(), self.table_m.data_ptr(), self.table_v.data_ptr(),
+                      self.table_last.data_ptr(), self._hp(), self.step_dev.data_ptr(), B, F, D, 1 if short_segments else 0, C.byref(hdr),
+                      tab.data_ptr(), wg_t.data_ptr(), wg_c.data_ptr(), n_wg), self._stream())
+            return
         L.launch("cdc_embed_segsum_lazy_update_dense", self.lib.cdc_embed_segsum_lazy_update_dense,
                  (d_out.data_ptr(), ws["seg"].data_ptr(), ws["perm"].data_ptr(), ws["cnt"].data_ptr(), ws["uniq"].data_ptr(),
                   self.table.data_ptr(), self.table_m.data_ptr(), self.table_v.data_ptr(), self.table_last.data_ptr(), self._hp(),
diff --git a/causal-domain-clustering-for-multi-domain-recommendation_amd/trainer.py b/causal-domain-clustering-for-multi-domain-recommendation_amd/trainer.py
--- a/causal-domain-clustering-for-multi-domain-recommendation_amd/trainer.py
+++ b/causal-domain-clustering-for-multi-domain-recommendation_amd/trainer.py
@@ -29,7 +29,8 @@
 
     def __init__(self, model, optimizer: FusedAdam, batch_size, mode="multi", use_graph=False, dist=None, sync_bn=True,
                  table_dist=None, shard_slack=1.5, train_mode=True, overlap=True, overlap_waves=2, sort_ahead=True, fuse_gather=False,
-                 defer_dw_reduce=None, global_rows=None, cap_rows=None, tower_one_launch=True, rows_dense_one_launch=True):
+                 defer_dw_reduce=None, global_rows=None, cap_rows=None, tower_one_launch=True, rows_dense_one_launch=True,
+                 stage_rows=True):
         self.model, self.opt, self.B, self.mode = model, optimizer, int(batch_size), mode
         self.lib = L.load()
         self.dist = dist
@@ -106,6 +107,10 @@
         D = self.emb.D
         self._fuse_gather_ok = lazy_one and bool(fuse_gather) and D % 4 == 0 and 64 % (D // 4) == 0
         self._ahead_ok = lazy_one and self._overlap_ok and bool(sort_ahead) and not self._fuse_gather_ok
+        self._stage_rows_ok = (lazy_one and bool(stage_rows) and not self._fuse_gather_ok and optimizer.can_stage_rows(D) and
+                               self.emb.out.grad.root.data_ptr() % 16 == 0)
+        if self._stage_rows_ok:
+            optimizer._row_state(self.B, self.emb.F, D)
         self._ahead_dp_ok = (self.dp_on and self.table_dist == "sharded" and bool(sort_ahead) and
                              (self.world > 1 or sort_ahead == "force"))
         self._stage_begins = lazy_one or self._ahead_dp_ok
@@ -231,7 +236,7 @@
                 self._reg()
                 return
             cur, nxt = f"a{p}", f"a{1 - p}"
-            bg, fused = self._overlap_ok, self._fuse_gather_ok
+            bg, fused, staged = self._overlap_ok, self._fuse_gather_ok, self._stage_rows_ok
             side = self._side_stream() if bg else main
             if bg:
                 side.wait_stream(main)
@@ -242,7 +247,7 @@
                     oh, ldh = plan.shadow_view(emb.out) if (plan.use_g2 and plan.has_shadow(emb.out)) else (None, 0)
                     opt.catchup_gather(B, F, D, cur, emb.out.ptr, oh, ldh)
                 else:
-                    opt.catchup(B, F, D, cur)
+                    opt.catchup(B, F, D, cur, stage=staged)
                 if bg:
                     rows_ready = torch.cuda.Event()
                     rows_ready.record(side)
@@ -262,12 +267,13 @@
             if self._rows_dense_one:
                 if bg:
                     main.wait_stream(side)
-                opt.rows_and_dense_step(emb.idx, emb.out.grad.root, B, F, D, plan.param_grads, plan._param_refs, plan.grad_slabs, tag=cur)
+                opt.rows_and_dense_step(emb.idx, emb.out.grad.root, B, F, D, plan.param_grads, plan._param_refs, plan.grad_slabs, tag=cur,
+                                        staged=staged)
             else:
                 opt.dense_step(plan.param_grads, plan._param_refs, plan.grad_slabs)
                 if bg:
                     main.wait_stream(side)
-                opt.table_step(emb.idx, emb.out.grad.root, B, F, D, tag=cur)
+                opt.table_step(emb.idx, emb.out.grad.root, B, F, D, tag=cur, staged=staged)
             self._reg()
         finally:
             self._towers_one_launch(False)
diff --git a/include/cdcmdr.h b/include/cdcmdr.h
--- a/include/cdcmdr.h
+++ b/include/cdcmdr.h
@@ -84,6 +84,13 @@
 int cdc_embed_segsum_lazy_update(const float* d_out, const int32_t* seg_start, const int32_t* perm, const int32_t* uniq_cnt,
                                  const int32_t* uniq_row, float* w, float* m, float* v, int32_t* last, cdc_adam_hp hp,
                                  const int32_t* step_dev, int64_t B, int32_t F, int32_t D, int32_t short_only, void* stream);
+int cdc_embed_lazy_catchup_stage(const int32_t* uniq_row, const int32_t* uniq_cnt, float* w, const float* m, const float* v,
+                                 int32_t* last, float* row_state, cdc_adam_hp hp, const int32_t* step_dev,
+                                 int64_t B, int32_t F, int32_t D, void* stream);
+int cdc_embed_segsum_lazy_update_staged(const float* d_out, const int32_t* seg_start, const int32_t* perm, const int32_t* uniq_cnt,
+                                        const int32_t* uniq_row, const float* row_state, float* w, float* m, float* v, int32_t* last,
+                                        cdc_adam_hp hp, const int32_t* step_dev, int64_t B, int32_t F, int32_t D, int32_t short_only,
+                                        void* stream);
 int cdc_embed_lazy_flush(float* w, float* m, float* v, int32_t* last, int64_t R, int32_t D,
                          cdc_adam_hp hp, const int32_t* step_dev, int32_t step_bias, int32_t period,
                          int32_t own_mod, int32_t own_rem, void* stream);
@@ -690,6 +697,12 @@
                                        const int32_t* step_dev, int64_t B, int32_t F, int32_t D, int32_t short_only,
                                        const cdc_adam_args* dense, const cdc_adam_tensor* tensors_dev, const int32_t* wg_tensor_dev,
                                        const int32_t* wg_chunk_dev, int32_t n_dense_workgroups, void* stream);
+int cdc_embed_segsum_lazy_update_dense_staged(const float* d_out, const int32_t* seg_start, const int32_t* perm, const int32_t* uniq_cnt,
+                                              const int32_t* uniq_row, const float* row_state, float* w, float* m, float* v,
+                                              int32_t* last, cdc_adam_hp hp, const int32_t* step_dev, int64_t B, int32_t F, int32_t D,
+                                              int32_t short_only, const cdc_adam_args* dense, const cdc_adam_tensor* tensors_dev,
+                                              const int32_t* wg_tensor_dev, const int32_t* wg_chunk_dev, int32_t n_dense_workgroups,
+                                              void* stream);
 
 typedef struct {
     int32_t n;
```

Measured after the change: 13.56 million samples/s, median of 6. No clear change (+0.5%).
